# CityU-AIM-Group/HTD

Hardware: AMD Instinct MI355X
Metric: images/sec (1333x800) HTD-R50 train step (higher is better)
Workload: dtype f32; 1 GPU; HTD ResNet-50 FPN fp32 train step fwd+bwd+SGD, batch 4/GPU @ 1333x800 (padded 1344x800), random-init weights, 2000 RPN proposals/img, 512 RoIs/img/stage; global_batch=4, parallelism=dp1, stage2_positives=168, proposals=random-init RPN (few positives: the regression branch is nearly idle)

## Files before the change

htd_amd/csrc/common.h:

```cpp
#pragma once
#include <hip/hip_runtime.h>
#include <stdint.h>
#include <stdio.h>
#include <string.h>

#include "../../include/htd_amd.h"

namespace htd {

void set_error(const char *fmt, ...);
int conv_math();

inline int check_launch(const char *what)
{
    hipError_t e = hipGetLastError();
    if (e != hipSuccess) {
        set_error("%s: launch failed: %s", what, hipGetErrorString(e));
        return HTD_ERR_LAUNCH;
    }
    return HTD_OK;
}

#define HTD_REQUIRE(cond, ...)               \
    do {                                     \
        if (!(cond)) {                       \
            htd::set_error(__VA_ARGS__);     \
            return HTD_ERR_ARG;              \
        }                                    \
    } while (0)

constexpr int kWave = 64;

__device__ __forceinline__ float wave_sum(float v)
{
#pragma unroll
    for (int o = 32; o > 0; o >>= 1) v += __shfl_xor(v, o, 64);
    return v;
}
__device__ __forceinline__ float wave_max(float v)
{
#pragma unroll
    for (int o = 32; o > 0; o >>= 1) v = fmaxf(v, __shfl_xor(v, o, 64));
    return v;
}

__device__ __forceinline__ unsigned mag_bits(float v) { return (v != v) ? 0x7fc00000u : (__float_as_uint(v) & 0x7fffffffu); }
__device__ __forceinline__ unsigned mag_bits4(unsigned mx, float4 v)
{
    return max(max(mx, max(mag_bits(v.x), mag_bits(v.y))), max(mag_bits(v.z), mag_bits(v.w)));
}
__device__ __forceinline__ void wave_mag_out(unsigned bits, float *out)
{
#pragma unroll
    for (int o = 32; o > 0; o >>= 1) bits = max(bits, (unsigned)__shfl_xor((int)bits, o, 64));
    if ((threadIdx.x & 63) == 0 && bits > *reinterpret_cast<volatile unsigned *>(out))
        __hip_atomic_fetch_max(reinterpret_cast<unsigned *>(out), bits, __ATOMIC_RELAXED, __HIP_MEMORY_SCOPE_AGENT);
}

inline int64_t ceil_div(int64_t a, int64_t b) { return (a + b - 1) / b; }

}
```

htd_amd/csrc/conv_fwd.hip:

```cpp
#include <algorithm>
#include <mutex>
#include <unordered_map>

#include <stdlib.h>

#include "common.h"

namespace {

using f32x16 = __attribute__((ext_vector_type(16))) float;
using bf16x8 = __attribute__((ext_vector_type(8))) __bf16;

using bf16x2 = __attribute__((ext_vector_type(2))) __bf16;
using f32x2 = __attribute__((ext_vector_type(2))) float;

__device__ __forceinline__ void split3x2(float a, float b, unsigned &h, unsigned &m, unsigned &l)
{
    union { bf16x2 v; unsigned u; } c;
    c.v = __builtin_convertvector(f32x2{a, b}, bf16x2);
    h = c.u;
    const float ra = a - __uint_as_float(h << 16), rb = b - __uint_as_float(h & 0xffff0000u);
    c.v = __builtin_convertvector(f32x2{ra, rb}, bf16x2);
    m = c.u;
    c.v = __builtin_convertvector(f32x2{ra - __uint_as_float(m << 16), rb - __uint_as_float(m & 0xffff0000u)}, bf16x2);
// ... 383 lines not shown
                    }
                }
#pragma unroll
                for (int u = 0; u < UB; ++u)
                    if (ok[u]) {
                        *reinterpret_cast<float4 *>(p.y + o[u]) = v[u];
                        omx = htd::mag_bits4(omx, v[u]);
                    }
            }
            if (i + 1 < TM) __syncthreads();
            continue;
        }
#pragma unroll
        for (int pass = 0; pass < NPASS; ++pass) {
            const int row = tid / V + pass * RPP;
            const int64_t m = m0 + ((row >> 5) * TM + i) * 32 + (row & 31);
            if (m >= p.M || n >= p.Co) continue;
            float4 v = *reinterpret_cast<const float4 *>(lds + row * T::EPI_STRIDE + c4 * 4);
            int64_t o;
            if constexpr (TAPS) {
                const unsigned mm = (unsigned)m, wo = mm % (unsigned)p.Wo, t = mm / (unsigned)p.Wo;
                const unsigned ho = t % (unsigned)p.Ho, b = t / (unsigned)p.Ho;
                o = (((int64_t)b * p.oH + p.o_h0 + p.o_step * (int)ho) * p.oW + p.o_w0 + p.o_step * (int)wo) * p.Co + n;
            } else
                o = m * p.Co + n;
            if (tail_split >= 0) {
                const int lrow = ((row >> 5) * TM + i) * 32 + (row & 31);
                float *dst = p.partial + ((int64_t)(bid - p.tail_first) * p.tail_splits + tail_split) * (T::BM * T::BN) +
                             lrow * T::BN + c4 * 4;
                *reinterpret_cast<float4 *>(dst) = v;
                continue;
            }
            if (p.splits > 1) {
                float *dst = p.partial + (int64_t)blockIdx.y * p.M * p.Co + o;
                if (vec_ok) *reinterpret_cast<float4 *>(dst) = v;
                else {
                    dst[0] = v.x;
                    if (n + 1 < p.Co) dst[1] = v.y;
                    if (n + 2 < p.Co) dst[2] = v.z;
                    if (n + 3 < p.Co) dst[3] = v.w;
                }
                continue;
            }
            if (vec_ok) {
                if (p.bias) {
                    const float4 bv = *reinterpret_cast<const float4 *>(p.bias + n);
                    v.x += bv.x; v.y += bv.y; v.z += bv.z; v.w += bv.w;
                }
                if (p.residual) {
                    int64_t ro = o;
                    if (p.res_H > 0) {
                        const unsigned mm = (unsigned)m, wo = mm % (unsigned)p.Wo, t = mm / (unsigned)p.Wo;
                        const unsigned ho = t % (unsigned)p.Ho, b = t / (unsigned)p.Ho;
                        const int rh = min((int)floorf(ho * p.res_sh), p.res_H - 1);
                        const int rw = min((int)floorf(wo * p.res_sw), p.res_W - 1);
                        ro = (((int64_t)b * p.res_H + rh) * p.res_W + rw) * p.Co + n;
                    }
                    const float4 rv = *reinterpret_cast<const float4 *>(p.residual + ro);
                    v.x += rv.x; v.y += rv.y; v.z += rv.z; v.w += rv.w;
                }
                if (p.relu) { v.x = fmaxf(v.x, 0.f); v.y = fmaxf(v.y, 0.f); v.z = fmaxf(v.z, 0.f); v.w = fmaxf(v.w, 0.f); }
                if (p.mask_src) {
                    const float4 mv = *reinterpret_cast<const float4 *>(p.mask_src + o);
                    v.x = mv.x > 0.f ? v.x : 0.f; v.y = mv.y > 0.f ? v.y : 0.f;
                    v.z = mv.z > 0.f ? v.z : 0.f; v.w = mv.w > 0.f ? v.w : 0.f;
                }
                *reinterpret_cast<float4 *>(p.y + o) = v;
                omx = htd::mag_bits4(omx, v);
            } else {
                auto put = [&](int e, float t) {
                    if (n + e >= p.Co) return;
                    t += p.bias ? p.bias[n + e] : 0.f;
                    if (p.residual) t += p.residual[o + e];
                    if (p.relu) t = fmaxf(t, 0.f);
                    if (p.mask_src) t = p.mask_src[o + e] > 0.f ? t : 0.f;
                    p.y[o + e] = t;
                    omx = max(omx, htd::mag_bits(t));
                };
                put(0, v.x); put(1, v.y); put(2, v.z); put(3, v.w);
            }
        }
        if (i + 1 < TM) __syncthreads();
    }
    if (p.amax_out != nullptr && tail_split < 0 && p.splits <= 1) htd::wave_mag_out(omx, p.amax_out);
}

__global__ __launch_bounds__(256) void conv_splitk_epilogue_kernel(ConvParams p)
{
    const int64_t total = p.M * p.Co;
    unsigned omx = 0u;
    for (int64_t o = (int64_t)blockIdx.x * blockDim.x + threadIdx.x; o < total; o += (int64_t)gridDim.x * blockDim.x) {
        float v = 0.f;
        for (int k = 0; k < p.splits; ++k) v += p.partial[(int64_t)k * total + o];
        const int n = (int)(o % p.Co);
        if (p.bias) v += p.bias[n];
        if (p.residual) {
            int64_t ro = o;
            if (p.res_H > 0) {
                const int64_t m = o / p.Co;
                const unsigned mm = (unsigned)m, wo = mm % (unsigned)p.Wo, t = mm / (unsigned)p.Wo;
                const unsigned ho = t % (unsigned)p.Ho, b = t / (unsigned)p.Ho;
                const int rh = min((int)floorf(ho * p.res_sh), p.res_H - 1);
                const int rw = min((int)floorf(wo * p.res_sw), p.res_W - 1);
                ro = (((int64_t)b * p.res_H + rh) * p.res_W + rw) * p.Co + n;
            }
            v += p.residual[ro];
        }
        if (p.relu) v = fmaxf(v, 0.f);
        if (p.mask_src) v = p.mask_src[o] > 0.f ? v : 0.f;
        p.y[o] = v;
        omx = max(omx, htd::mag_bits(v));
    }
    if (p.amax_out != nullptr) htd::wave_mag_out(omx, p.amax_out);
}

__global__ __launch_bounds__(256) void conv_tail_epilogue_kernel(ConvParams p, int BM, int BN)
{
    const int64_t per_tile = (int64_t)BM * BN, total = (int64_t)(p.mt * p.nt - p.tail_first) * per_tile;
    unsigned omx = 0u;
    for (int64_t e = (int64_t)blockIdx.x * blockDim.x + threadIdx.x; e < total; e += (int64_t)gridDim.x * blockDim.x) {
        const int t = (int)(e / per_tile), within = (int)(e - (int64_t)t * per_tile);
        const int tile = p.tail_first + t, tile_m = tile / p.nt, tile_n = tile % p.nt;
        const int64_t m = (int64_t)tile_m * BM + within / BN;
        const int n = tile_n * BN + within % BN;
        if (m >= p.M || n >= p.Co) continue;
        const float *src = p.partial + (int64_t)t * p.tail_splits * per_tile + within;
        float v = 0.f;
        for (int k = 0; k < p.tail_splits; ++k) v += src[(int64_t)k * per_tile];
        const int64_t o = m * p.Co + n;
        if (p.bias) v += p.bias[n];
        if (p.residual) {
            int64_t ro = o;
            if (p.res_H > 0) {
                const unsigned mm = (unsigned)m, wo = mm % (unsigned)p.Wo, tt = mm / (unsigned)p.Wo;
                const unsigned ho = tt % (unsigned)p.Ho, b = tt / (unsigned)p.Ho;
                const int rh = min((int)floorf(ho * p.res_sh), p.res_H - 1);
                const int rw = min((int)floorf(wo * p.res_sw), p.res_W - 1);
                ro = (((int64_t)b * p.res_H + rh) * p.res_W + rw) * p.Co + n;
            }
            v += p.residual[ro];
        }
        if (p.relu) v = fmaxf(v, 0.f);
        if (p.mask_src) v = p.mask_src[o] > 0.f ? v : 0.f;
        p.y[o] = v;
        omx = max(omx, htd::mag_bits(v));
    }
    if (p.amax_out != nullptr) htd::wave_mag_out(omx, p.amax_out);
}

int g_conv_math = getenv("HTD_CONV_MATH") ? atoi(getenv("HTD_CONV_MATH")) : 1;

template <int WGM, int WGN, int TM, int TN>
void launch_cfg(const ConvParams &p, unsigned blocks, hipStream_t s)
{
    const dim3 grid(blocks, p.splits);
    const bool x3 = g_conv_math == 1;
    if (p.ntaps > 0) {
        if (p.Ci % 16 == 0) {
            if (x3) hipLaunchKernelGGL((conv_igemm_kernel<16, WGM, WGN, TM, TN, true, true>), grid, dim3(256), 0, s, p);
            else hipLaunchKernelGGL((conv_igemm_kernel<16, WGM, WGN, TM, TN, true>), grid, dim3(256), 0, s, p);
        } else
            hipLaunchKernelGGL((conv_igemm_kernel<8, WGM, WGN, TM, TN, true>), grid, dim3(256), 0, s, p);
    } else if (p.Ci % 32 == 0) {
        if (x3) hipLaunchKernelGGL((conv_igemm_kernel<32, WGM, WGN, TM, TN, false, true>), grid, dim3(256), 0, s, p);
        else hipLaunchKernelGGL((conv_igemm_kernel<32, WGM, WGN, TM, TN, false>), grid, dim3(256), 0, s, p);
    } else if (p.Ci % 16 == 0) {
        if (x3) hipLaunchKernelGGL((conv_igemm_kernel<16, WGM, WGN, TM, TN, false, true>), grid, dim3(256), 0, s, p);
        else hipLaunchKernelGGL((conv_igemm_kernel<16, WGM, WGN, TM, TN, false>), grid, dim3(256), 0, s, p);
    } else
        hipLaunchKernelGGL((conv_igemm_kernel<8, WGM, WGN, TM, TN, false>), grid, dim3(256), 0, s, p);
}

int plan_splits(int64_t M, int Co, int Ci, int taps)
{
    const int bk = Ci % 32 == 0 ? 32 : (Ci % 16 == 0 ? 16 : 8);
    const int total_slices = taps * (Ci / bk);
    const int64_t tiles = htd::ceil_div(M, 128) * htd::ceil_div(Co, 64);
    if (tiles <= 0 || tiles >= 384 || total_slices < 16) return 1;
    int64_t want = htd::ceil_div(768, tiles);
    want = std::min<int64_t>(want, total_slices / 8);
    return (int)std::max<int64_t>(1, std::min<int64_t>(want, 16));
}

struct TileCfg { int bm, bn; };
constexpr TileCfg kTileCfg[] = {{64, 64}, {128, 32}, {128, 64}, {128, 128}, {128, 64}, {64, 128}};
constexpr int kNumTileCfg = 6;

static const bool g_tune = getenv("HTD_CONV_TUNE") != nullptr;
int forced_tile()
{
    if (!g_tune) return -1;
    const char *e = getenv("HTD_CONV_FORCE_TILE");
    const int v = e ? atoi(e) : -1;
    return (v >= 0 && v < kNumTileCfg) ? v : -1;
}

static float tile_score(int cfg, int64_t M, int Co, int K, int splits)
{
    const int bm = kTileCfg[cfg].bm, bn = kTileCfg[cfg].bn;
    const int64_t tiles = htd::ceil_div(M, bm) * htd::ceil_div(Co, bn);
    const bool long_k = K >= 1024;
    float base;
    if (g_conv_math == 1) {
        switch (cfg) {
        case 3: base = 1.00f; break;
        case 4: base = long_k ? 0.86f : 0.90f; break;
        case 5: base = long_k ? 0.88f : 0.94f; break;
        default: base = long_k ? 0.72f : 0.82f; break;
        }
    } else {
        switch (cfg) {
        case 3: base = long_k ? 1.00f : 0.90f; break;
        case 4: base = long_k ? 0.98f : 0.97f; break;
        case 5: base = long_k ? 0.98f : 0.98f; break;
        default: base = long_k ? 0.86f : (K >= 512 ? 0.90f : 0.95f); break;
        }
    }
    const float w = (float)(tiles * splits) / 256.f;
    float quant;
    if (w >= 7.f) quant = w / ceilf(w);
    else if (w >= 3.f) quant = 0.97f;
    else quant = w / ceilf(w);
    const float useful = (float)((double)M * Co / ((double)tiles * bm * bn));
    return base * quant * useful;
}

struct TileKey {
    int64_t M;
    int Co, Ci, taps, epi;
    bool operator==(const TileKey &o) const { return M == o.M && Co == o.Co && Ci == o.Ci && taps == o.taps && epi == o.epi; }
// ... 18 lines not shown
    return it == g_tile_table.end() ? -1 : it->second;
}

int choose_tile(int64_t M, int Co, int Ci, int taps, int epi, int splits, int &bm, int &bn)
{
    const int K = taps * Ci;
    int cfg = forced_tile();
    if (cfg < 0 && epi >= 0) cfg = table_tile(M, Co, Ci, taps, epi);
    if (cfg >= 0 && Co <= 64 && kTileCfg[cfg].bn > 64) cfg = -1;
    if (cfg < 0) {
        if (Co <= 32) cfg = 1;
        else if (Co <= 64) cfg = (htd::ceil_div(M, 128) * htd::ceil_div(Co, 64) < 4400 && M >= 2048) ? 0 : 2;
        else {
            static const int cand[4] = {3, 4, 5, 0};
            float best = -1.f;
            for (int c : cand) {
                const float sc = tile_score(c, M, Co, K, splits);
                if (sc > best * 1.005f) { best = sc; cfg = c; }
            }
        }
    }
    bm = kTileCfg[cfg].bm;
    bn = kTileCfg[cfg].bn;
    return cfg;
}

static const bool g_no_tail = getenv("HTD_CONV_NO_TAIL") != nullptr;
int plan_tail(int64_t M, int Co, int Ci, int taps, int bm, int bn, int &tail_splits, int &tail_sps)
{
    tail_splits = tail_sps = 0;
    if (g_no_tail || (Co & 3)) return 0;
    const int bk = Ci % 32 == 0 ? 32 : (Ci % 16 == 0 ? 16 : 8);
    const int total_slices = taps * (Ci / bk);
    const int64_t tiles = htd::ceil_div(M, bm) * htd::ceil_div(Co, bn);
    const int64_t rem = tiles % 256, whole = tiles - rem;
    if (tiles < 256 * 3 || tiles >= 256 * 7 || rem == 0 || rem > 128 || total_slices < 8) return 0;
    int want = (int)std::min<int64_t>(16, std::max<int64_t>(2, (256 + rem / 2) / rem));
    want = std::min(want, total_slices / 4);
    if (want < 2) return 0;
    tail_sps = (int)htd::ceil_div(total_slices, want);
    tail_splits = (int)htd::ceil_div(total_slices, tail_sps);
    return (int)whole;
}

int launch_conv(ConvParams p, hipStream_t s, void *workspace)
{
    const int bk = (p.Ci % 32 == 0 && p.ntaps == 0) ? 32 : (p.Ci % 16 == 0 ? 16 : 8);
    const int total_slices = (p.ntaps > 0 ? p.ntaps : p.kh * p.kw) * (p.Ci / bk);
    p.splits = (workspace && p.ntaps == 0) ? plan_splits(p.M, p.Co, p.Ci, p.kh * p.kw) : 1;
    p.slices_per_split = (int)htd::ceil_div(total_slices, p.splits);
    p.splits = (int)htd::ceil_div(total_slices, p.slices_per_split);
    int bm, bn;
    const int epi = (p.ntaps > 0 || p.w_bstride > 0) ? -1 : ((p.residual ? 1 : 0) | (p.mask_src ? 2 : 0));
    const int cfg = choose_tile(p.M, p.Co, p.Ci, p.ntaps > 0 ? p.ntaps : p.kh * p.kw, epi, p.splits, bm, bn);
    p.mt = (int)htd::ceil_div(p.M, bm);
    p.nt = (int)htd::ceil_div(p.Co, bn);
    const int64_t blocks = (int64_t)p.mt * p.nt;
    HTD_REQUIRE(blocks > 0 && blocks < (1ll << 31), "conv2d: bad grid");
    HTD_REQUIRE((int64_t)p.B * p.Hx * p.Wx * p.Ci < (1ll << 31) && (int64_t)p.Co * p.kh * p.kw * p.Ci < (1ll << 31) &&
                    p.M < (1ll << 31),
                "conv2d: operand larger than 2^31 elements (32-bit element offsets)");
    p.partial = (float *)workspace;
    static const int cmajor_env = getenv("HTD_CONV_CMAJOR") ? atoi(getenv("HTD_CONV_CMAJOR")) : 1;
    p.cmajor = (p.ntaps == 0 && p.kh * p.kw > 1) ? cmajor_env : 0;
    unsigned launch_blocks = (unsigned)blocks;
    p.tail_first = p.tail_splits = p.tail_sps = 0;
    if (workspace && p.ntaps == 0 && p.splits == 1 && p.w_bstride == 0) {
        const int whole = plan_tail(p.M, p.Co, p.Ci, p.kh * p.kw, bm, bn, p.tail_splits, p.tail_sps);
        if (p.tail_splits > 0) {
            p.tail_first = whole;
            launch_blocks = (unsigned)(whole + (blocks - whole) * p.tail_splits);
        }
    }
    switch (cfg) {
    case 0: launch_cfg<2, 2, 1, 1>(p, launch_blocks, s); break;
    case 1: launch_cfg<4, 1, 1, 1>(p, launch_blocks, s); break;
    case 2: launch_cfg<4, 1, 1, 2>(p, launch_blocks, s); break;
    case 3: launch_cfg<2, 2, 2, 2>(p, launch_blocks, s); break;
    case 4: launch_cfg<2, 2, 2, 1>(p, launch_blocks, s); break;
    default: launch_cfg<2, 2, 1, 2>(p, launch_blocks, s); break;
    }
    if (p.tail_splits > 0) {
        const int64_t elems = (blocks - p.tail_first) * (int64_t)bm * bn;
        hipLaunchKernelGGL(conv_tail_epilogue_kernel, dim3((unsigned)htd::ceil_div(elems, 256)), dim3(256), 0, s, p, bm, bn);
    }
    if (p.splits > 1) {
        const unsigned rb = (unsigned)std::min<int64_t>(htd::ceil_div(p.M * p.Co, 256), 4096);
        hipLaunchKernelGGL(conv_splitk_epilogue_kernel, dim3(rb), dim3(256), 0, s, p);
    }
    return htd::check_launch("conv2d");
}

}

namespace htd {
int conv_math() { return g_conv_math; }
}

static int conv2d_fwd_impl(const float *x, const float *w, const float *bias, const float *residual, int res_h, int res_w, float *y,
                           int B, int H, int W, int Ci, int Co, int kh, int kw, int stride, int pad, int dil, int relu,
                           float *amax_out, void *workspace, void *stream)
{
    HTD_REQUIRE((res_h > 0) == (res_w > 0) && res_h >= 0 && (res_h == 0 || ((Co & 3) == 0 && residual)),
                "conv2d_fwd: bad residual up-sampling arguments");
    HTD_REQUIRE(B > 0 && H > 0 && W > 0 && Ci > 0 && Co > 0 && kh > 0 && kw > 0 && stride > 0 && dil > 0 && pad >= 0,
                "conv2d_fwd: bad sizes B=%d H=%d W=%d Ci=%d Co=%d k=%dx%d s=%d p=%d d=%d", B, H, W, Ci, Co, kh, kw,
                stride, pad, dil);
    HTD_REQUIRE(Ci % 8 == 0, "conv2d_fwd: Ci=%d must be a multiple of 8 (pad the stem input to 8 channels)", Ci);
    HTD_REQUIRE(x && w && y, "conv2d_fwd: null pointer");
    ConvParams p{};
    p.x = x; p.w = w; p.bias = bias; p.residual = residual; p.mask_src = nullptr; p.y = y;
    p.B = B; p.H = H; p.W = W; p.Ci = Ci; p.Co = Co; p.kh = kh; p.kw = kw; p.stride = stride; p.pad = pad; p.dil = dil;
    p.Ho = (H + 2 * pad - (dil * (kh - 1) + 1)) / stride + 1;
    p.Wo = (W + 2 * pad - (dil * (kw - 1) + 1)) / stride + 1;
    HTD_REQUIRE(p.Ho > 0 && p.Wo > 0, "conv2d_fwd: empty output");
    p.Hx = H; p.Wx = W; p.relu = relu;
    p.amax_out = amax_out;
    p.M = (int64_t)B * p.Ho * p.Wo;
    if (res_h > 0) {
        p.res_H = res_h; p.res_W = res_w;
        p.res_sh = (float)res_h / (float)p.Ho; p.res_sw = (float)res_w / (float)p.Wo;
    }
    return launch_conv(p, (hipStream_t)stream, workspace);
}

extern "C" int htd_conv2d_fwd(const float *x, const float *w, const float *bias, const float *residual, int res_h,
                              int res_w, float *y, int B, int H, int W, int Ci, int Co, int kh, int kw, int stride,
                              int pad, int dil, int relu, void *workspace, void *stream)
{
    return conv2d_fwd_impl(x, w, bias, residual, res_h, res_w, y, B, H, W, Ci, Co, kh, kw, stride, pad, dil, relu, nullptr, workspace,
                           stream);
}

extern "C" int htd_conv2d_fwd_amax(const float *x, const float *w, const float *bias, const float *residual, int res_h, int res_w,
                                   float *y, float *amax_out, int B, int H, int W, int Ci, int Co, int kh, int kw, int stride, int pad,
                                   int dil, int relu, void *workspace, void *stream)
{
    HTD_REQUIRE(amax_out, "conv2d_fwd: null maximum");
    return conv2d_fwd_impl(x, w, bias, residual, res_h, res_w, y, B, H, W, Ci, Co, kh, kw, stride, pad, dil, relu, amax_out, workspace,
                           stream);
}

extern "C" int64_t htd_conv2d_workspace_bytes(int64_t M, int Co, int Ci, int kh, int kw)
{
    const int splits = plan_splits(M, Co, Ci, kh * kw);
    if (splits > 1) return (int64_t)splits * M * Co * 4;
    int64_t need = 0;
    for (int epi = 0; epi < 4; ++epi) {
        int bm, bn, ts, tsps;
        choose_tile(M, Co, Ci, kh * kw, epi, 1, bm, bn);
        const int whole = plan_tail(M, Co, Ci, kh * kw, bm, bn, ts, tsps);
        if (ts == 0) continue;
        const int64_t tiles = htd::ceil_div(M, bm) * htd::ceil_div(Co, bn);
        need = std::max(need, (tiles - whole) * ts * (int64_t)bm * bn * 4);
    }
    return need;
}

extern "C" int htd_conv2d_tile_table_set(int64_t M, int Co, int Ci, int taps, int epi, int cfg)
{
    HTD_REQUIRE(M > 0 && Co > 0 && Ci > 0 && taps > 0 && epi >= 0 && epi < 4 && cfg < kNumTileCfg,
                "tile_table_set: bad entry M=%lld Co=%d Ci=%d taps=%d epi=%d cfg=%d", (long long)M, Co, Ci, taps, epi, cfg);
    std::lock_guard<std::mutex> lock(g_tile_mutex);
    if (cfg < 0) g_tile_table.erase(TileKey{M, Co, Ci, taps, epi});
    else g_tile_table[TileKey{M, Co, Ci, taps, epi}] = cfg;
    return HTD_OK;
}

extern "C" int htd_conv2d_tile_table_clear()
{
// ... 191 lines not shown
```

htd_amd/csrc/conv_wgrad.hip:

```cpp
#include <algorithm>

#include "common.h"

namespace {

using f32x16 = __attribute__((ext_vector_type(16))) float;

__device__ __forceinline__ float4 keep4(bool ok, float4 v)
{
    return make_float4(ok ? v.x : 0.f, ok ? v.y : 0.f, ok ? v.z : 0.f, ok ? v.w : 0.f);
}

struct WgradParams {
    const float *x, *gy;
    float *out;
    float *bias_out;
    int B, H, W, Ci, Co, kh, kw, stride, pad, dil, Ho, Wo;
    int64_t K;
    int Ntot;
    int mt, nt, splits;
    int64_t slices_per_split;
    const float *amax_x, *amax_g;
};

// ... 1174 lines not shown
    const int fcol = lane & 31, fhalf = lane >> 5;
    const int ci = ci0 + wn * 32 + fcol;
    if (ci < p.Ci) {
#pragma unroll
        for (int t = 0; t < 3; ++t) {
            const int n = (ky * 3 + t) * p.Ci + ci;
#pragma unroll
            for (int i = 0; i < TM; ++i)
#pragma unroll
                for (int r = 0; r < 16; ++r) {
                    const int m = m0 + wm * TM * 32 + i * 32 + (r & 3) + 8 * (r >> 2) + 4 * fhalf;
                    if (m < p.Co) out[(int64_t)m * p.Ntot + n] = H2 ? acc[t][i][r] * sg_inv * sx_inv : acc[t][i][r];
                }
        }
    }
}

__global__ __launch_bounds__(256) void splitk_reduce_kernel(const float *__restrict__ ws, float *__restrict__ out,
                                                            int64_t n, int splits, const float *__restrict__ ws2 = nullptr,
                                                            float *__restrict__ out2 = nullptr, int n2 = 0, int acc = 0)
{
    const int extra = out2 ? (n2 + 255) / 256 : 0;
    if ((int)blockIdx.x >= (int)gridDim.x - extra) {
        const int i = ((int)blockIdx.x - ((int)gridDim.x - extra)) * 256 + threadIdx.x;
        if (i < n2) {
            float s = acc ? out2[i] : 0.f;
            int k = 0;
            for (; k + 3 < splits; k += 4) {
                const float a = ws2[(int64_t)k * n2 + i], b = ws2[(int64_t)(k + 1) * n2 + i];
                const float c = ws2[(int64_t)(k + 2) * n2 + i], d = ws2[(int64_t)(k + 3) * n2 + i];
                s += a; s += b; s += c; s += d;
            }
            for (; k < splits; ++k) s += ws2[(int64_t)k * n2 + i];
            out2[i] = s;
        }
        return;
    }
    const unsigned main_blocks = gridDim.x - extra;
    const int64_t n4 = (n & 3) == 0 ? (n >> 2) : 0;
    for (int64_t i = (int64_t)blockIdx.x * blockDim.x + threadIdx.x; i < n4; i += (int64_t)main_blocks * blockDim.x) {
        float4 s = acc ? *reinterpret_cast<const float4 *>(out + i * 4) : make_float4(0.f, 0.f, 0.f, 0.f);
        int k = 0;
        for (; k + 3 < splits; k += 4) {
            float4 v[4];
#pragma unroll
            for (int u = 0; u < 4; ++u) v[u] = *reinterpret_cast<const float4 *>(ws + (int64_t)(k + u) * n + i * 4);
#pragma unroll
            for (int u = 0; u < 4; ++u) { s.x += v[u].x; s.y += v[u].y; s.z += v[u].z; s.w += v[u].w; }
        }
        for (; k < splits; ++k) {
            const float4 v = *reinterpret_cast<const float4 *>(ws + (int64_t)k * n + i * 4);
            s.x += v.x; s.y += v.y; s.z += v.z; s.w += v.w;
        }
        *reinterpret_cast<float4 *>(out + i * 4) = s;
    }
    if (blockIdx.x == 0)
        for (int64_t i = n4 * 4 + threadIdx.x; i < n; i += blockDim.x) {
            float s = acc ? out[i] : 0.f;
            for (int k = 0; k < splits; ++k) s += ws[(int64_t)k * n + i];
            out[i] = s;
        }
}

__global__ __launch_bounds__(256) void reduce_rows_kernel(const float *__restrict__ ws, float *__restrict__ out, int n,
                                                          int rows)
{
    __shared__ float red[16][17];
    const int col = threadIdx.x & 15, grp = threadIdx.x >> 4;
    const int c = blockIdx.x * 16 + col;
    float s = 0.f;
    if (c < n)
        for (int k = grp; k < rows; k += 16) s += ws[(int64_t)k * n + c];
    red[grp][col] = s;
    __syncthreads();
    if (grp == 0 && c < n) {
        float t = red[0][col];
#pragma unroll
        for (int g = 1; g < 16; ++g) t += red[g][col];
        out[c] = t;
    }
}

using htd::mag_bits;
using htd::wave_mag_out;

__global__ __launch_bounds__(256) void colsum_mask_kernel(const float *__restrict__ g, const float *__restrict__ y,
                                                          float *__restrict__ gm, float *__restrict__ partial,
                                                          int64_t rows, int C, int64_t rows_per_block, float *__restrict__ amax_out)
{
    const int c = blockIdx.y * 256 + threadIdx.x;
    const int64_t r0 = (int64_t)blockIdx.x * rows_per_block, r1 = min(rows, r0 + rows_per_block);
    float s = 0.f;
    unsigned mx = 0u;
    if (c < C)
        for (int64_t r = r0; r < r1; ++r) {
            float v = g[r * C + c];
            if (y) {
                v = y[r * C + c] > 0.f ? v : 0.f;
                gm[r * C + c] = v;
            }
            mx = max(mx, mag_bits(v));
            s += v;
        }
    if (amax_out) wave_mag_out(mx, amax_out);
    if (partial && c < C) partial[(int64_t)blockIdx.x * C + c] = s;
}

__global__ __launch_bounds__(256) void colsum_mask_vec_kernel(const float *__restrict__ g, const float *__restrict__ y,
                                                              float *__restrict__ gm, float *__restrict__ partial,
                                                              int64_t rows, int C, int64_t rows_per_block,
                                                              float *__restrict__ amax_out)
{
    __shared__ float4 red[256];
    unsigned mx = 0u;
    const int C4 = C >> 2;
    const int cbase = blockIdx.y * 256;
    const int cw = min(256, C4 - cbase);
    const int R = 256 / cw;
    const int c4 = threadIdx.x % cw, rsub = threadIdx.x / cw;
    const int64_t r0 = (int64_t)blockIdx.x * rows_per_block, r1 = min(rows, r0 + rows_per_block);
    float4 s = make_float4(0.f, 0.f, 0.f, 0.f);
    if (rsub < R) {
        int64_t r = r0 + rsub;
        for (; r + 3 * (int64_t)R < r1; r += 4 * (int64_t)R) {
            float4 v[4], yv[4];
#pragma unroll
            for (int u = 0; u < 4; ++u) {
                const int64_t o = (r + u * (int64_t)R) * C + (int64_t)(cbase + c4) * 4;
                v[u] = *reinterpret_cast<const float4 *>(g + o);
                if (y) yv[u] = *reinterpret_cast<const float4 *>(y + o);
            }
#pragma unroll
            for (int u = 0; u < 4; ++u) {
                if (y) {
                    const int64_t o = (r + u * (int64_t)R) * C + (int64_t)(cbase + c4) * 4;
                    v[u].x = yv[u].x > 0.f ? v[u].x : 0.f; v[u].y = yv[u].y > 0.f ? v[u].y : 0.f;
                    v[u].z = yv[u].z > 0.f ? v[u].z : 0.f; v[u].w = yv[u].w > 0.f ? v[u].w : 0.f;
                    *reinterpret_cast<float4 *>(gm + o) = v[u];
                }
                mx = htd::mag_bits4(mx, v[u]);
                s.x += v[u].x; s.y += v[u].y; s.z += v[u].z; s.w += v[u].w;
            }
        }
        for (; r < r1; r += R) {
            const int64_t o = r * C + (int64_t)(cbase + c4) * 4;
            float4 v = *reinterpret_cast<const float4 *>(g + o);
            if (y) {
                const float4 yv = *reinterpret_cast<const float4 *>(y + o);
                v.x = yv.x > 0.f ? v.x : 0.f; v.y = yv.y > 0.f ? v.y : 0.f;
                v.z = yv.z > 0.f ? v.z : 0.f; v.w = yv.w > 0.f ? v.w : 0.f;
                *reinterpret_cast<float4 *>(gm + o) = v;
            }
            mx = htd::mag_bits4(mx, v);
            s.x += v.x; s.y += v.y; s.z += v.z; s.w += v.w;
        }
    }
    if (amax_out) wave_mag_out(mx, amax_out);
    if (!partial) return;
    red[threadIdx.x] = s;
    __syncthreads();
    if (rsub == 0) {
        for (int k = 1; k < R; ++k) {
            const float4 t = red[k * cw + c4];
            s.x += t.x; s.y += t.y; s.z += t.z; s.w += t.w;
        }
        *reinterpret_cast<float4 *>(partial + (int64_t)blockIdx.x * C + (int64_t)(cbase + c4) * 4) = s;
    }
}

struct Cfg { int splits; int mt, nt; int bm, bn; };

template <int WGM, int WGN, int TM, int TN>
void launch_wgrad(int pix, bool covec, dim3 grid, hipStream_t s, const WgradParams &p)
{
#define HTD_WGRAD_CASE(PIX, CV)                                                                                   \
    if (pix == PIX && covec == CV) {                                                                               \
        hipLaunchKernelGGL((conv_wgrad_kernel<WGM, WGN, TM, TN, PIX, CV>), grid, dim3(256), 0, s, p);             \
        return;                                                                                                    \
    }
    HTD_WGRAD_CASE(PIX_POINTWISE, true) HTD_WGRAD_CASE(PIX_WIDE, true) HTD_WGRAD_CASE(PIX_GENERAL, true)
    HTD_WGRAD_CASE(PIX_POINTWISE, false) HTD_WGRAD_CASE(PIX_WIDE, false) HTD_WGRAD_CASE(PIX_GENERAL, false)
#undef HTD_WGRAD_CASE
}

Cfg choose(int Co, int Ntot, int64_t K)
{
    Cfg c;
    c.bm = Co <= 32 ? 32 : 128;
    c.bn = 128;
    c.mt = (int)htd::ceil_div(Co, c.bm);
    c.nt = (int)htd::ceil_div(Ntot, c.bn);
    const int64_t slices = htd::ceil_div(K, BKW);
    static const int units = getenv("HTD_WGRAD_UNITS") ? atoi(getenv("HTD_WGRAD_UNITS")) : 1536;
    int64_t want = htd::ceil_div(units, (int64_t)c.mt * c.nt);
    const int64_t tiles = (int64_t)c.mt * c.nt;
    int64_t cap = std::max<int64_t>(1, slices / 20);
    if (tiles * cap < 256)
        cap = std::max(cap, std::min<int64_t>(htd::ceil_div(256, tiles), std::max<int64_t>(1, slices / 5)));
    want = std::min<int64_t>(want, cap);
    c.splits = (int)std::max<int64_t>(1, std::min<int64_t>(want, 192));
    if (c.splits >= 6) c.splits = (c.splits + 7) / 8 * 8;
    static const int forced = getenv("HTD_WGRAD_SPLITS") ? atoi(getenv("HTD_WGRAD_SPLITS")) : 0;
    if (forced > 0) c.splits = (int)std::min<int64_t>(forced, slices);
    return c;
}

static const bool g_wgrad_x3h_off = getenv("HTD_WGRAD_X3H") != nullptr && atoi(getenv("HTD_WGRAD_X3H")) == 0;
bool x3h_takes(int Ci, int Co, int kh, int kw, int stride, int pad, int dil)
{
    return !g_wgrad_x3h_off && kh == 3 && kw == 3 && stride == 1 && pad == 1 && dil == 1 && Co >= 64 && (Co & 3) == 0 &&
           Ci >= 32 && (Ci & 3) == 0;
}
int x3h_splits(int B, int H, int W, int Ci, int Co)
{
    const int64_t tiles = htd::ceil_div(Co, 128) * htd::ceil_div(Ci, 64) * 3;
    const int64_t slices = htd::ceil_div((int64_t)B * H * (W + 1), XH_KS);
    static const int target = getenv("HTD_WGRAD_X3H_UNITS") ? atoi(getenv("HTD_WGRAD_X3H_UNITS")) : 768;
    int64_t want = htd::ceil_div(target, tiles);
    int64_t cap = std::max<int64_t>(1, slices / 8);
    if (tiles * cap < 256) cap = std::max(cap, std::min<int64_t>(htd::ceil_div(256, tiles), std::max<int64_t>(1, slices / 4)));
    want = std::min<int64_t>(want, cap);
    int splits = (int)std::max<int64_t>(1, std::min<int64_t>(want, 128));
    if (splits >= 6) splits = (splits + 7) / 8 * 8;
    static const int forced = getenv("HTD_WGRAD_X3H_SPLITS") ? atoi(getenv("HTD_WGRAD_X3H_SPLITS")) : 0;
    if (forced > 0) splits = (int)std::min<int64_t>(forced, std::max<int64_t>(1, slices / 2));
    return splits;
}

}

int g_wgrad_math = -1;

extern "C" int64_t htd_conv2d_wgrad_workspace_bytes(int B, int H, int W, int Ci, int Co, int kh, int kw, int stride,
                                                    int pad, int dil)
{
    const int Ho = (H + 2 * pad - (dil * (kh - 1) + 1)) / stride + 1;
    const int Wo = (W + 2 * pad - (dil * (kw - 1) + 1)) / stride + 1;
    const Cfg c = choose(Co, kh * kw * Ci, (int64_t)B * Ho * Wo);
    int splits = c.splits;
    if (x3h_takes(Ci, Co, kh, kw, stride, pad, dil)) splits = std::max(splits, x3h_splits(B, H, W, Ci, Co));
// ... 200 lines not shown
```

htd_amd/csrc/conv_x3.hip:

```cpp
#include <algorithm>
#include <mutex>
#include <type_traits>
#include <unordered_map>

#include <stdlib.h>

#include "common.h"

namespace {

using f32x16 = __attribute__((ext_vector_type(16))) float;
using bf16x8 = __attribute__((ext_vector_type(8))) __bf16;
using bf16x2 = __attribute__((ext_vector_type(2))) __bf16;
using f32x2 = __attribute__((ext_vector_type(2))) float;
using f32x4 = __attribute__((ext_vector_type(4))) float;

using f16x8 = __attribute__((ext_vector_type(8))) _Float16;
using f16x2 = __attribute__((ext_vector_type(2))) _Float16;

constexpr int XK = 16;
constexpr int NCH = 6;

struct H2Scale { float s, inv; };
__device__ __forceinline__ H2Scale h2_scale(const float *amax)
// ... 11 lines not shown
    const f32x2 back = __builtin_convertvector(c.v, f32x2);
    c.v = __builtin_convertvector(f32x2{a - back[0], b - back[1]}, f16x2);
    l = c.u;
}

__device__ __forceinline__ void split3x2(float a, float b, unsigned &h, unsigned &m, unsigned &l)
{
    union { bf16x2 v; unsigned u; } c;
    c.v = __builtin_convertvector(f32x2{a, b}, bf16x2);
    h = c.u;
    const float ra = a - __uint_as_float(h << 16), rb = b - __uint_as_float(h & 0xffff0000u);
    c.v = __builtin_convertvector(f32x2{ra, rb}, bf16x2);
    m = c.u;
    c.v = __builtin_convertvector(f32x2{ra - __uint_as_float(m << 16), rb - __uint_as_float(m & 0xffff0000u)}, bf16x2);
    l = c.u;
}

#ifndef HTD_X3P_EARLY
#define HTD_X3P_EARLY 1
#endif
#ifndef HTD_X3H_NB
#define HTD_X3H_NB 2
#endif
#ifndef HTD_X3H_FRAG_FIRST
#define HTD_X3H_FRAG_FIRST 1
#endif
#ifndef HTD_X3H_OCC4
#define HTD_X3H_OCC4 0
#endif

template <int N>
__device__ __forceinline__ void wait_vm()
{
    asm volatile("s_waitcnt vmcnt(%0)" ::"n"(N) : "memory");
}
__device__ __forceinline__ void landed(f32x4 &a) { asm volatile("" : "+v"(a)::"memory"); }

__device__ __forceinline__ void lds_dma16(const void *src, unsigned lds_dst)
{
    unsigned keep;
    asm volatile("s_mov_b32 %0, m0\n\ts_mov_b32 m0, %2\n\ts_nop 0\n\tglobal_load_lds_dwordx4 %1, off\n\ts_mov_b32 m0, %0"
                 : "=&s"(keep)
                 : "v"(src), "s"(lds_dst)
                 : "memory");
}

using u32x2 = __attribute__((ext_vector_type(2))) unsigned;
template <int OFF>
__device__ __forceinline__ void lds_store8(unsigned addr, unsigned lo, unsigned hi)
{
    const u32x2 v = {lo, hi};
    asm volatile("ds_write_b64 %0, %1 offset:%2" ::"v"(addr), "v"(v), "n"(OFF) : "memory");
}

struct X3Params {
    const float *x;
    const uint4 *wp;
    const float *bias, *residual, *mask_src;
    float *y;
    int Hx, Wx;
    int Ho, Wo;
    int Ci, Co, Cop;
    int kh;
    int stride;
    int ntl;
    int tl_dy[9], tl_dx[9], tl_w[9];
    int o_step, o_h0, o_w0, oH, oW;
    int relu;
    int res_H, res_W;
    float res_sh, res_sw;
    int64_t M;
    int mt, nt;
    int ncs;
    int tiles_a, splits_a, sps_a, splits_b, sps_b;
    int64_t m_rem0;
    float *partial;
    const uint4 *xp;
    uint4 *yp;
    int64_t xp_rows, yp_rows;
    const float *amax, *wscale;
    float *amax_out;
};

__device__ __forceinline__ void block_absmax_out(float mx, float *out, float *red, unsigned seen)
{
    unsigned bits = (mx != mx) ? 0x7fc00000u : __float_as_uint(mx);
    for (int o = 32; o > 0; o >>= 1) bits = max(bits, (unsigned)__shfl_xor((int)bits, o));
    __syncthreads();
    if ((threadIdx.x & 63) == 0) reinterpret_cast<unsigned *>(red)[threadIdx.x >> 6] = bits;
    __syncthreads();
    if (threadIdx.x == 0) {
        const unsigned *r = reinterpret_cast<const unsigned *>(red);
        bits = max(max(r[0], r[1]), max(r[2], r[3]));
        if (bits > seen) __hip_atomic_fetch_max(reinterpret_cast<unsigned *>(out), bits, __ATOMIC_RELAXED, __HIP_MEMORY_SCOPE_AGENT);
    }
}
__device__ __forceinline__ void wave_absmax_out(float mx, float *out, unsigned seen)
{
    unsigned bits = (mx != mx) ? 0x7fc00000u : __float_as_uint(mx);
    for (int o = 32; o > 0; o >>= 1) bits = max(bits, (unsigned)__shfl_xor((int)bits, o));
    if ((threadIdx.x & 63) == 0 && bits > seen)
        __hip_atomic_fetch_max(reinterpret_cast<unsigned *>(out), bits, __ATOMIC_RELAXED, __HIP_MEMORY_SCOPE_AGENT);
}
__device__ __forceinline__ float absmax4(float mx, float4 v)
{
    const float m = fmaxf(fmaxf(fabsf(v.x), fabsf(v.y)), fmaxf(fabsf(v.z), fabsf(v.w)));
    const bool nan = (v.x != v.x) | (v.y != v.y) | (v.z != v.z) | (v.w != v.w);
    return nan ? __uint_as_float(0x7fc00000u) : ((mx != mx) ? mx : fmaxf(mx, m));
}

__device__ __forceinline__ void emit_planes4(uint4 *yp, int64_t rows, int64_t m, int n, float4 v)
{
    unsigned h0, m0, l0, h1, m1, l1;
    split3x2(v.x, v.y, h0, m0, l0);
    split3x2(v.z, v.w, h1, m1, l1);
    char *d = reinterpret_cast<char *>(yp + ((int64_t)(n >> 4) * NCH + ((n >> 3) & 1)) * rows + m) + ((n >> 2) & 1) * 8;
    *reinterpret_cast<uint2 *>(d) = make_uint2(h0, h1);
    *reinterpret_cast<uint2 *>(d + 2 * rows * 16) = make_uint2(m0, m1);
    *reinterpret_cast<uint2 *>(d + 4 * rows * 16) = make_uint2(l0, l1);
}

template <int BM, int KW>
struct Geo {
    static constexpr int RUN = BM + KW - 1;
    static constexpr int PITCH = ((RUN + 1 + 3) / 8) * 8 + 4;
    static constexpr int PASSES = (RUN + 63) / 64;
};

__device__ __forceinline__ int64_t x3_out_off(const X3Params &p, int64_t m, int n)
{
    if (p.o_step == 0) return m * p.Co + n;
    const unsigned mm = (unsigned)m, wo = mm % (unsigned)p.Wo, t = mm / (unsigned)p.Wo;
    const unsigned ho = t % (unsigned)p.Ho, b = t / (unsigned)p.Ho;
    return (((int64_t)b * p.oH + p.o_h0 + p.o_step * (int)ho) * p.oW + p.o_w0 + p.o_step * (int)wo) * p.Co + n;
}

template <int WGM, int WGN, int TM, int TN, bool MF16, typename Acc>
__device__ __forceinline__ void x3_epilogue(const X3Params &p, Acc &acc, uint4 *lds, int64_t m0, int n0, bool part, bool region_b,
                                            int split)
{
    constexpr int BN = WGN * TN * 32;
    constexpr int EPI_STRIDE = BN + 4, EPI_ROWS = WGM * 32;
    constexpr int RBLK = MF16 ? 16 : 32;
    constexpr int CB = TN * 32 / RBLK;
    const int tid = threadIdx.x, lane = tid & 63, wave = tid >> 6;
    const int wm = wave / WGN, wn = wave % WGN;
    const int frow = lane & 31, fhalf = lane >> 5;
    const int lrow = MF16 ? (lane & 15) : frow;
    const int kg = lane >> 4;
    float *le = reinterpret_cast<float *>(lds);
    const bool vec_ok = (p.Co & 3) == 0;
    constexpr int V = BN / 4, RPP = 256 / V;
    float omax = 0.f;
    const unsigned oseen = (p.amax_out != nullptr && !part) ? *reinterpret_cast<const volatile unsigned *>(p.amax_out) : 0u;
    const bool scaled = p.wscale != nullptr;
    float4 cscale = make_float4(1.f, 1.f, 1.f, 1.f);
    if (scaled) {
        const float ia = h2_scale(p.amax).inv;
        const float4 w4 = *reinterpret_cast<const float4 *>(p.wscale + n0 + (tid % V) * 4);
        cscale = make_float4(w4.x * ia, w4.y * ia, w4.z * ia, w4.w * ia);
    }
#pragma unroll
    for (int i = 0; i < TM; ++i) {
        if constexpr (MF16) {
#pragma unroll
            for (int ib = 0; ib < 2; ++ib)
#pragma unroll
                for (int j = 0; j < CB; ++j)
#pragma unroll
                    for (int r = 0; r < 4; ++r)
                        le[(wm * 32 + ib * 16 + 4 * kg + r) * EPI_STRIDE + wn * TN * 32 + j * 16 + lrow] = acc[2 * i + ib][j][r];
        } else {
#pragma unroll
            for (int j = 0; j < TN; ++j)
#pragma unroll
                for (int r = 0; r < 16; ++r) {
                    const int row = wm * 32 + (r & 3) + 8 * (r >> 2) + 4 * fhalf;
                    le[row * EPI_STRIDE + (wn * TN + j) * 32 + frow] = acc[i][j][r];
                }
        }
        __syncthreads();
        const int c4 = tid % V;
        const int n = n0 + c4 * 4;
        constexpr int NPASS = EPI_ROWS / RPP;
        if (vec_ok && !part && p.res_H == 0) {
            const bool col_ok = n < p.Co;
            float4 bv = make_float4(0.f, 0.f, 0.f, 0.f);
            if (p.bias != nullptr && col_ok) bv = *reinterpret_cast<const float4 *>(p.bias + n);
            constexpr int UB = NPASS < 4 ? NPASS : 4;
#pragma unroll
            for (int pass0 = 0; pass0 < NPASS; pass0 += UB) {
                float4 v[UB], rv[UB], mv[UB];
                int64_t o[UB];
                bool ok[UB];
#pragma unroll
                for (int u = 0; u < UB; ++u) {
                    const int row = tid / V + (pass0 + u) * RPP;
                    const int64_t m = m0 + ((row >> 5) * TM + i) * 32 + (row & 31);
                    ok[u] = m < p.M && col_ok;
                    o[u] = x3_out_off(p, ok[u] ? m : 0, n) & -(int64_t)ok[u];
                    v[u] = *reinterpret_cast<const float4 *>(le + row * EPI_STRIDE + c4 * 4);
                    if (scaled) { v[u].x *= cscale.x; v[u].y *= cscale.y; v[u].z *= cscale.z; v[u].w *= cscale.w; }
                }
                if (p.residual != nullptr) {
#pragma unroll
                    for (int u = 0; u < UB; ++u) rv[u] = *reinterpret_cast<const float4 *>(p.residual + o[u]);
                }
                if (p.mask_src != nullptr) {
#pragma unroll
                    for (int u = 0; u < UB; ++u) mv[u] = *reinterpret_cast<const float4 *>(p.mask_src + o[u]);
                }
#pragma unroll
                for (int u = 0; u < UB; ++u) { v[u].x += bv.x; v[u].y += bv.y; v[u].z += bv.z; v[u].w += bv.w; }
                if (p.residual != nullptr) {
#pragma unroll
                    for (int u = 0; u < UB; ++u) { v[u].x += rv[u].x; v[u].y += rv[u].y; v[u].z += rv[u].z; v[u].w += rv[u].w; }
                }
                if (p.relu) {
#pragma unroll
                    for (int u = 0; u < UB; ++u) {
                        v[u].x = fmaxf(v[u].x, 0.f); v[u].y = fmaxf(v[u].y, 0.f); v[u].z = fmaxf(v[u].z, 0.f); v[u].w = fmaxf(v[u].w, 0.f);
                    }
                }
                if (p.mask_src != nullptr) {
#pragma unroll
                    for (int u = 0; u < UB; ++u) {
                        v[u].x = mv[u].x > 0.f ? v[u].x : 0.f; v[u].y = mv[u].y > 0.f ? v[u].y : 0.f;
                        v[u].z = mv[u].z > 0.f ? v[u].z : 0.f; v[u].w = mv[u].w > 0.f ? v[u].w : 0.f;
                    }
                }
#pragma unroll
                for (int u = 0; u < UB; ++u)
                    if (ok[u]) {
                        *reinterpret_cast<float4 *>(p.y + o[u]) = v[u];
                        omax = absmax4(omax, v[u]);
                    }
                if (p.yp != nullptr) {
#pragma unroll
                    for (int u = 0; u < UB; ++u) {
                        const int row = tid / V + (pass0 + u) * RPP;
                        if (ok[u]) emit_planes4(p.yp, p.yp_rows, m0 + ((row >> 5) * TM + i) * 32 + (row & 31), n, v[u]);
                    }
                }
            }
            if (i + 1 < TM) __syncthreads();
            continue;
        }
#pragma unroll
        for (int pass = 0; pass < NPASS; ++pass) {
            const int row = tid / V + pass * RPP;
            const int64_t m = m0 + ((row >> 5) * TM + i) * 32 + (row & 31);
            if (m >= p.M || n >= p.Co) continue;
            float4 v = *reinterpret_cast<const float4 *>(le + row * EPI_STRIDE + c4 * 4);
            if (scaled) { v.x *= cscale.x; v.y *= cscale.y; v.z *= cscale.z; v.w *= cscale.w; }
            const int64_t o = x3_out_off(p, m, n);
            if (part) {
                float *dst = region_b ? p.partial + (p.splits_a > 1 ? (int64_t)p.splits_a * p.m_rem0 * p.Co : 0) +
                                            ((int64_t)split * (p.M - p.m_rem0) + (m - p.m_rem0)) * p.Co + n
                                      : p.partial + ((int64_t)split * p.m_rem0 + m) * p.Co + n;
                if (vec_ok) *reinterpret_cast<float4 *>(dst) = v;
                else {
                    dst[0] = v.x;
                    if (n + 1 < p.Co) dst[1] = v.y;
                    if (n + 2 < p.Co) dst[2] = v.z;
                    if (n + 3 < p.Co) dst[3] = v.w;
                }
                continue;
            }
            if (vec_ok) {
                if (p.bias) {
                    const float4 bv = *reinterpret_cast<const float4 *>(p.bias + n);
                    v.x += bv.x; v.y += bv.y; v.z += bv.z; v.w += bv.w;
                }
                if (p.residual) {
                    int64_t ro = o;
                    if (p.res_H > 0) {
                        const unsigned mm = (unsigned)m, wo = mm % (unsigned)p.Wo, t = mm / (unsigned)p.Wo;
                        const unsigned ho = t % (unsigned)p.Ho, b = t / (unsigned)p.Ho;
                        const int rh = min((int)floorf(ho * p.res_sh), p.res_H - 1);
                        const int rw = min((int)floorf(wo * p.res_sw), p.res_W - 1);
                        ro = (((int64_t)b * p.res_H + rh) * p.res_W + rw) * p.Co + n;
                    }
                    const float4 rv = *reinterpret_cast<const float4 *>(p.residual + ro);
                    v.x += rv.x; v.y += rv.y; v.z += rv.z; v.w += rv.w;
                }
                if (p.relu) { v.x = fmaxf(v.x, 0.f); v.y = fmaxf(v.y, 0.f); v.z = fmaxf(v.z, 0.f); v.w = fmaxf(v.w, 0.f); }
                if (p.mask_src) {
                    const float4 mv = *reinterpret_cast<const float4 *>(p.mask_src + o);
                    v.x = mv.x > 0.f ? v.x : 0.f; v.y = mv.y > 0.f ? v.y : 0.f;
                    v.z = mv.z > 0.f ? v.z : 0.f; v.w = mv.w > 0.f ? v.w : 0.f;
                }
                *reinterpret_cast<float4 *>(p.y + o) = v;
                omax = absmax4(omax, v);
                if (p.yp != nullptr) emit_planes4(p.yp, p.yp_rows, m, n, v);
            } else {
                auto put = [&](int e, float t) {
                    if (n + e >= p.Co) return;
                    t += p.bias ? p.bias[n + e] : 0.f;
                    if (p.residual) t += p.residual[o + e];
                    if (p.relu) t = fmaxf(t, 0.f);
                    if (p.mask_src) t = p.mask_src[o + e] > 0.f ? t : 0.f;
                    p.y[o + e] = t;
                    omax = absmax4(omax, make_float4(t, 0.f, 0.f, 0.f));
                };
                put(0, v.x); put(1, v.y); put(2, v.z); put(3, v.w);
            }
        }
        if (i + 1 < TM) __syncthreads();
    }
    if (p.amax_out != nullptr && !part) block_absmax_out(omax, p.amax_out, le, oseen);
}

template <int WGM, int WGN, int TM, int TN, int KW, int NB, bool H2 = false>
constexpr int x3p_occupancy()
{
    constexpr int BM = WGM * TM * 32, BN = WGN * TN * 32;
    constexpr int NCHL = H2 ? 4 : NCH;
    constexpr int main_bytes = (2 * NCHL * Geo<BM, KW>::PITCH + NB * NCHL * BN) * 16;
    constexpr int epi_bytes = WGM * 32 * (BN + 4) * 4;
    constexpr int by_lds = 163840 / (main_bytes > epi_bytes ? main_bytes : epi_bytes);
    constexpr int by_regs = TM * TN >= 4 ? (H2 && HTD_X3H_OCC4 ? 4 : 3) : 4;
    return by_lds < by_regs ? by_lds : by_regs;
}

template <int WGM, int WGN, int TM, int TN, int KW, bool MF16, int NB, bool H2 = false>
__global__ __launch_bounds__(256, (x3p_occupancy<WGM, WGN, TM, TN, KW, NB, H2>())) void conv_x3p_kernel(X3Params p)
{
    static_assert(!(H2 && MF16), "H2: 32x32x16 form only");
    constexpr int NCHL = H2 ? 4 : NCH;
    constexpr int BM = WGM * TM * 32, BN = WGN * TN * 32;
    using G = Geo<BM, KW>;
    constexpr int PADX = (KW - 1) / 2;
    constexpr int A_VEC = NCHL * G::PITCH;
    constexpr int B_VEC = NCHL * BN;
    constexpr int MAIN_VEC = 2 * A_VEC + NB * B_VEC;
    constexpr int EPI_STRIDE = BN + 4, EPI_ROWS = WGM * 32;
    constexpr int EPI_VEC = EPI_ROWS * EPI_STRIDE / 4;
    constexpr int LDS_VEC = MAIN_VEC > EPI_VEC ? MAIN_VEC : EPI_VEC;
    __shared__ uint4 lds[LDS_VEC];
    uint4 *const lA = lds, *const lB = lds + 2 * A_VEC;
    const unsigned lds_a0 = (unsigned)(size_t)(__attribute__((address_space(3))) void *)lA;

    int bid = blockIdx.x, split = 0, sps = 0;
    bool part = false;
    const bool region_b = bid >= p.tiles_a * p.splits_a;
    if (region_b) {
        const int r = bid - p.tiles_a * p.splits_a;
        bid = p.tiles_a + r / p.splits_b;
        split = r % p.splits_b;
        part = p.splits_b > 1;
        sps = p.sps_b;
    } else if (p.splits_a > 1) {
        split = bid % p.splits_a;
        bid = bid / p.splits_a;
        part = true;
        sps = p.sps_a;
    } else {
        const int q = p.tiles_a / 8, r = p.tiles_a % 8, xcd = bid % 8, idx = bid / 8;
        bid = (xcd < r ? xcd * (q + 1) : r * (q + 1) + (xcd - r) * q) + idx;
    }
    const int tile_m = bid / p.nt, tile_n = bid % p.nt;
    const int64_t m0 = (int64_t)tile_m * BM;
    const int n0 = tile_n * BN;

    const int tid = threadIdx.x, lane = tid & 63, wave = tid >> 6;
    const int wm = wave / WGN, wn = wave % WGN;
    const int frow = lane & 31, fhalf = lane >> 5;
    const int PADY = (p.kh - 1) / 2;

    const int vcol = tid & 3, vrow = tid >> 2;
    const int a_g0 = (int)m0 + vrow - PADX;
    unsigned a_off[KW > 1 ? 1 : G::PASSES];
    bool a_in[KW > 1 ? 1 : G::PASSES];
    unsigned a_tm[KW > 1 ? 1 : G::PASSES];
    if constexpr (KW > 1) {
        a_off[0] = (unsigned)a_g0 * (unsigned)p.Ci + vcol * 4;
        a_in[0] = true;
        a_tm[0] = 0u;
    } else {
#pragma unroll
        for (int i = 0; i < G::PASSES; ++i) {
            const int64_t m = m0 + vrow + 64 * i;
            a_in[i] = vrow + 64 * i < G::RUN && m < p.M;
            const unsigned mm = a_in[i] ? (unsigned)m : 0u;
            const unsigned wo = mm % (unsigned)p.Wo, t = mm / (unsigned)p.Wo;
            const unsigned ho = t % (unsigned)p.Ho, b = t / (unsigned)p.Ho;
            a_off[i] = ((b * (unsigned)p.Hx + ho * (unsigned)p.stride) * (unsigned)p.Wx + wo * (unsigned)p.stride) *
                           (unsigned)p.Ci + vcol * 4;
            unsigned tm = 0x1ffu;
            if (p.ntl > 0) {
                tm = 0u;
                const int hb = (int)(ho * (unsigned)p.stride), wb = (int)(wo * (unsigned)p.stride);
                for (int q = 0; q < p.ntl; ++q)
// ... 462 lines not shown

    using acc_t = typename std::conditional<MF16, f32x4, f32x16>::type;
    acc_t acc[RB][CB];
#pragma unroll
    for (int i = 0; i < RB; ++i)
#pragma unroll
        for (int j = 0; j < CB; ++j)
#pragma unroll
            for (int r = 0; r < (MF16 ? 4 : 16); ++r) acc[i][j][r] = 0.f;

    auto mma = [&](int stage) __attribute__((always_inline)) {
        const char *la = reinterpret_cast<const char *>(lA + stage * A_VEC);
        const char *lb = reinterpret_cast<const char *>(lB + stage * B_VEC);
        if constexpr (MF16) {
            bf16x8 fa01[RB], fa02[RB];
#pragma unroll
            for (int i = 0; i < RB; ++i) {
                fa01[i] = *reinterpret_cast<const bf16x8 *>(la + a_c0 + i * 16 * 16);
                fa02[i] = *reinterpret_cast<const bf16x8 *>(la + a_c1 + i * 16 * 16);
            }
#pragma unroll
            for (int j = 0; j < CB; ++j) {
                const bf16x8 fb01 = *reinterpret_cast<const bf16x8 *>(lb + b_c0 + j * 16 * 16);
                const bf16x8 fb10 = *reinterpret_cast<const bf16x8 *>(lb + b_c1 + j * 16 * 16);
                const bf16x8 fb20 = *reinterpret_cast<const bf16x8 *>(lb + b_c2 + j * 16 * 16);
#pragma unroll
                for (int i = 0; i < RB; ++i) {
                    acc[i][j] = __builtin_amdgcn_mfma_f32_16x16x32_bf16(fa02[i], fb20, acc[i][j], 0, 0, 0);
                    acc[i][j] = __builtin_amdgcn_mfma_f32_16x16x32_bf16(fa01[i], fb10, acc[i][j], 0, 0, 0);
                    acc[i][j] = __builtin_amdgcn_mfma_f32_16x16x32_bf16(fa01[i], fb01, acc[i][j], 0, 0, 0);
                }
            }
        } else {
            bf16x8 fa[RB][3], fb[CB][3];
#pragma unroll
            for (int i = 0; i < RB; ++i)
#pragma unroll
                for (int q = 0; q < 3; ++q) fa[i][q] = *reinterpret_cast<const bf16x8 *>(la + a_c0 + i * 32 * 16 + q * 2 * BM * 16);
#pragma unroll
            for (int j = 0; j < CB; ++j)
#pragma unroll
                for (int q = 0; q < 3; ++q) fb[j][q] = *reinterpret_cast<const bf16x8 *>(lb + b_c0 + j * 32 * 16 + q * 2 * BN * 16);
#pragma unroll
            for (int i = 0; i < RB; ++i)
#pragma unroll
                for (int j = 0; j < CB; ++j) {
                    acc[i][j] = __builtin_amdgcn_mfma_f32_32x32x16_bf16(fa[i][2], fb[j][0], acc[i][j], 0, 0, 0);
                    acc[i][j] = __builtin_amdgcn_mfma_f32_32x32x16_bf16(fa[i][0], fb[j][2], acc[i][j], 0, 0, 0);
                    acc[i][j] = __builtin_amdgcn_mfma_f32_32x32x16_bf16(fa[i][1], fb[j][1], acc[i][j], 0, 0, 0);
                    acc[i][j] = __builtin_amdgcn_mfma_f32_32x32x16_bf16(fa[i][1], fb[j][0], acc[i][j], 0, 0, 0);
                    acc[i][j] = __builtin_amdgcn_mfma_f32_32x32x16_bf16(fa[i][0], fb[j][1], acc[i][j], 0, 0, 0);
                    acc[i][j] = __builtin_amdgcn_mfma_f32_32x32x16_bf16(fa[i][0], fb[j][0], acc[i][j], 0, 0, 0);
                }
        }
    };

    constexpr int KEEP = (NS - 2) * (NI / 4);
#pragma unroll
    for (int d = 0; d < NS - 1; ++d)
        if (s_begin + d < s_end) issue(s_begin + d, d);
    if (s_begin + NS - 2 < s_end) wait_vm<KEEP>();
    else wait_vm<0>();
    lds_barrier();
    int stage = 0, pstage = NS - 1;
#pragma unroll 1
    for (int s = s_begin; s < s_end; ++s) {
        const bool more = s + NS - 1 < s_end;
        if (more) issue(s + NS - 1, pstage);
        mma(stage);
        if (more) wait_vm<KEEP>();
        else wait_vm<0>();
        lds_barrier();
        stage = stage + 1 == NS ? 0 : stage + 1;
        pstage = pstage + 1 == NS ? 0 : pstage + 1;
    }
    x3_epilogue<WGM, WGN, TM, TN, MF16>(p, acc, lds, m0, n0, part, region_b, split);
}

__global__ __launch_bounds__(256) void conv_x3p_splitk_epilogue_kernel(X3Params p)
{
    const int64_t lo = p.splits_a > 1 ? 0 : p.m_rem0 * p.Co, hi = p.splits_b > 1 ? p.M * p.Co : p.m_rem0 * p.Co;
    const int64_t na = p.m_rem0 * p.Co, nb = (p.M - p.m_rem0) * p.Co;
    const float *pb = p.partial + (p.splits_a > 1 ? (int64_t)p.splits_a * na : 0);
    float omax = 0.f;
    const unsigned oseen = p.amax_out != nullptr ? *reinterpret_cast<const volatile unsigned *>(p.amax_out) : 0u;
    for (int64_t o = lo + (int64_t)blockIdx.x * blockDim.x + threadIdx.x; o < hi; o += (int64_t)gridDim.x * blockDim.x) {
        float v = 0.f;
        if (o < na) {
            for (int k = 0; k < p.splits_a; ++k) v += p.partial[(int64_t)k * na + o];
        } else {
            for (int k = 0; k < p.splits_b; ++k) v += pb[(int64_t)k * nb + (o - na)];
        }
        const int n = (int)(o % p.Co);
        if (p.bias) v += p.bias[n];
        if (p.residual) {
            int64_t ro = p.o_step == 0 ? o : x3_out_off(p, o / p.Co, n);
            if (p.res_H > 0) {
                const int64_t m = o / p.Co;
                const unsigned mm = (unsigned)m, wo = mm % (unsigned)p.Wo, t = mm / (unsigned)p.Wo;
                const unsigned ho = t % (unsigned)p.Ho, b = t / (unsigned)p.Ho;
                const int rh = min((int)floorf(ho * p.res_sh), p.res_H - 1);
                const int rw = min((int)floorf(wo * p.res_sw), p.res_W - 1);
                ro = (((int64_t)b * p.res_H + rh) * p.res_W + rw) * p.Co + n;
            }
            v += p.residual[ro];
        }
        if (p.relu) v = fmaxf(v, 0.f);
        const int64_t oo = p.o_step == 0 ? o : x3_out_off(p, o / p.Co, n);
        if (p.mask_src) v = p.mask_src[oo] > 0.f ? v : 0.f;
        p.y[oo] = v;
        omax = absmax4(omax, make_float4(v, 0.f, 0.f, 0.f));
    }
    __shared__ float ored[4];
    if (p.amax_out != nullptr) block_absmax_out(omax, p.amax_out, ored, oseen);
}

__global__ __launch_bounds__(256) void conv_x3p_splitk_epilogue_vec_kernel(X3Params p)
{
    const int C4 = p.Co >> 2;
    const int64_t lo = p.splits_a > 1 ? 0 : p.m_rem0 * C4, hi = p.splits_b > 1 ? p.M * C4 : p.m_rem0 * C4;
    const int64_t na = p.m_rem0 * C4, nb = (p.M - p.m_rem0) * C4;
    const float4 *pa = reinterpret_cast<const float4 *>(p.partial);
    const float4 *pb = pa + (p.splits_a > 1 ? (int64_t)p.splits_a * na : 0);
    float omax = 0.f;
    const unsigned oseen = p.amax_out != nullptr ? *reinterpret_cast<const volatile unsigned *>(p.amax_out) : 0u;
    for (int64_t q = lo + (int64_t)blockIdx.x * blockDim.x + threadIdx.x; q < hi; q += (int64_t)gridDim.x * blockDim.x) {
        float4 v = make_float4(0.f, 0.f, 0.f, 0.f);
        const bool in_a = q < na;
        const float4 *src = in_a ? pa + q : pb + (q - na);
        const int64_t stride = in_a ? na : nb;
        const int splits = in_a ? p.splits_a : p.splits_b;
#pragma unroll 4
        for (int k = 0; k < splits; ++k) {
            const float4 t = src[(int64_t)k * stride];
            v.x += t.x; v.y += t.y; v.z += t.z; v.w += t.w;
        }
        const unsigned m = (unsigned)(q / C4), n = (unsigned)(q - (int64_t)m * C4) * 4u;
        const int64_t o = x3_out_off(p, (int64_t)m, (int)n);
        if (p.bias) {
            const float4 bv = *reinterpret_cast<const float4 *>(p.bias + n);
            v.x += bv.x; v.y += bv.y; v.z += bv.z; v.w += bv.w;
        }
        if (p.residual) {
            int64_t ro = o;
            if (p.res_H > 0) {
                const unsigned wo = m % (unsigned)p.Wo, t = m / (unsigned)p.Wo;
                const unsigned ho = t % (unsigned)p.Ho, b = t / (unsigned)p.Ho;
                const int rh = min((int)floorf(ho * p.res_sh), p.res_H - 1);
                const int rw = min((int)floorf(wo * p.res_sw), p.res_W - 1);
                ro = (((int64_t)b * p.res_H + rh) * p.res_W + rw) * p.Co + n;
            }
            const float4 rv = *reinterpret_cast<const float4 *>(p.residual + ro);
            v.x += rv.x; v.y += rv.y; v.z += rv.z; v.w += rv.w;
        }
        if (p.relu) { v.x = fmaxf(v.x, 0.f); v.y = fmaxf(v.y, 0.f); v.z = fmaxf(v.z, 0.f); v.w = fmaxf(v.w, 0.f); }
        if (p.mask_src) {
            const float4 mv = *reinterpret_cast<const float4 *>(p.mask_src + o);
            v.x = mv.x > 0.f ? v.x : 0.f; v.y = mv.y > 0.f ? v.y : 0.f;
            v.z = mv.z > 0.f ? v.z : 0.f; v.w = mv.w > 0.f ? v.w : 0.f;
        }
        *reinterpret_cast<float4 *>(p.y + o) = v;
        omax = absmax4(omax, v);
        if (p.yp != nullptr) emit_planes4(p.yp, p.yp_rows, (int64_t)m, (int)n, v);
    }
    __shared__ float ored[4];
    if (p.amax_out != nullptr) block_absmax_out(omax, p.amax_out, ored, oseen);
}

__device__ __forceinline__ void x3_planes_element(const float *__restrict__ w, uint4 *__restrict__ out, int Co, int taps,
                                                  int Ci, int Np, int transposed, int64_t e)
{
    const int N = transposed ? Ci : Co, K = transposed ? Co : Ci;
    const int ncs = K / XK;
    const int n = (int)(e % Np);
    const int64_t t2 = e / Np;
    const int cs = (int)(t2 % ncs), tap = (int)(t2 / ncs);
    float v[XK];
    if (n < N) {
        if (!transposed) {
            const float4 *src = reinterpret_cast<const float4 *>(w + ((int64_t)n * taps + tap) * Ci + cs * XK);
#pragma unroll
            for (int q = 0; q < 4; ++q) {
                const float4 f = src[q];
                v[4 * q] = f.x; v[4 * q + 1] = f.y; v[4 * q + 2] = f.z; v[4 * q + 3] = f.w;
            }
        } else {
#pragma unroll
            for (int k = 0; k < XK; ++k) v[k] = w[((int64_t)(cs * XK + k) * taps + (taps - 1 - tap)) * Ci + n];
        }
    } else {
#pragma unroll
        for (int k = 0; k < XK; ++k) v[k] = 0.f;
    }
    unsigned pl[3][8];
#pragma unroll
    for (int k = 0; k < 8; ++k) split3x2(v[2 * k], v[2 * k + 1], pl[0][k], pl[1][k], pl[2][k]);
    uint4 *dst = out + ((int64_t)(tap * ncs + cs) * NCH) * Np + n;
#pragma unroll
    for (int q = 0; q < 3; ++q)
#pragma unroll
        for (int h = 0; h < 2; ++h)
            dst[(int64_t)(q * 2 + h) * Np] = make_uint4(pl[q][4 * h], pl[q][4 * h + 1], pl[q][4 * h + 2], pl[q][4 * h + 3]);
}

__global__ __launch_bounds__(256) void x3_planes_kernel(const float *__restrict__ w, uint4 *__restrict__ out, int Co, int taps,
                                                        int Ci, int Np, int transposed)
{
    const int K = transposed ? Co : Ci;
    const int64_t total = (int64_t)taps * (K / XK) * Np;
    for (int64_t e = (int64_t)blockIdx.x * 256 + threadIdx.x; e < total; e += (int64_t)gridDim.x * 256)
        x3_planes_element(w, out, Co, taps, Ci, Np, transposed, e);
}

struct PlanesDesc {
    const float *w;
    uint4 *out;
    int Co, taps, Ci, transposed;
    int64_t block0;
};

__global__ __launch_bounds__(256) void x3_planes_many_kernel(const PlanesDesc *__restrict__ descs, int n)
{
    int lo = 0, hi = n - 1;
    const int64_t b = blockIdx.x;
    while (lo < hi) {
        const int mid = (lo + hi + 1) >> 1;
        if (descs[mid].block0 <= b) lo = mid;
        else hi = mid - 1;
    }
    const PlanesDesc d = descs[lo];
    const int N = d.transposed ? d.Ci : d.Co, K = d.transposed ? d.Co : d.Ci;
    const int Np = ((N + 127) / 128) * 128;
    const int64_t total = (int64_t)d.taps * (K / XK) * Np;
    const int64_t e = (b - d.block0) * 256 + threadIdx.x;
    if (e < total) x3_planes_element(d.w, d.out, d.Co, d.taps, d.Ci, Np, d.transposed, e);
}

inline int planes_np(int N) { return (int)htd::ceil_div(N, 128) * 128; }

constexpr int H2_ECH = 1024;
__host__ __device__ inline int h2_chunks(int taps, int K) { return (taps * K + H2_ECH - 1) / H2_ECH; }

__device__ __forceinline__ void x3h_rowmax_part(const float *__restrict__ w, float *__restrict__ part, int Co, int taps, int Ci, int Np,
                                                int transposed, int n0, int chunk, float *red )
{
    const int N = transposed ? Ci : Co, K = transposed ? Co : Ci;
    const int lane = threadIdx.x & 63, wave = threadIdx.x >> 6;
    const int e0 = chunk * H2_ECH, e1 = min(taps * K, e0 + H2_ECH);
    if (transposed) {
// ... 361 lines not shown
        if (kw == 1) hipLaunchKernelGGL((conv_x3p_kernel<2, 2, TM, TN, 1, true, NB>), grid, dim3(256), 0, s, p);
        else hipLaunchKernelGGL((conv_x3p_kernel<2, 2, TM, TN, 3, true, NB>), grid, dim3(256), 0, s, p);
    }
}

template <int TM, int TN>
void launch_tile(const X3Params &p, int kw, dim3 grid, hipStream_t s)
{
#ifdef HTD_X3P_DEEP
    const int nb = x3p_nb();
    if (nb == 3) return launch_tile_nb<TM, TN, 3>(p, kw, grid, s);
    if (nb >= 4) return launch_tile_nb<TM, TN, 4>(p, kw, grid, s);
#endif
    launch_tile_nb<TM, TN, 2>(p, kw, grid, s);
}

static const int g_x3q_mfma = getenv("HTD_X3Q_MFMA") ? atoi(getenv("HTD_X3Q_MFMA")) : 0;
static const int g_x3q_ns = getenv("HTD_X3Q_NS") ? atoi(getenv("HTD_X3Q_NS")) : 0;
int x3q_env(const char *name, int at_load)
{
    if (!g_x3p_tune) return at_load;
    const char *e = getenv(name);
    return e ? atoi(e) : 0;
}

template <int TM, int TN>
void launch_tile_q(const X3Params &p, dim3 grid, hipStream_t s)
{
    const int mf = x3q_env("HTD_X3Q_MFMA", g_x3q_mfma), ns = x3q_env("HTD_X3Q_NS", g_x3q_ns);
    if (mf != 32) {
        if (ns == 3) hipLaunchKernelGGL((conv_x3q_kernel<2, 2, TM, TN, true, 3>), grid, dim3(256), 0, s, p);
        else hipLaunchKernelGGL((conv_x3q_kernel<2, 2, TM, TN, true, 2>), grid, dim3(256), 0, s, p);
    } else {
        if (ns == 3) hipLaunchKernelGGL((conv_x3q_kernel<2, 2, TM, TN, false, 3>), grid, dim3(256), 0, s, p);
        else hipLaunchKernelGGL((conv_x3q_kernel<2, 2, TM, TN, false, 2>), grid, dim3(256), 0, s, p);
    }
}

int launch_x3p(X3Params p, int kw, hipStream_t s, void *workspace)
{
    const int total_steps = p.ncs * p.kh;
    const int epi = (p.residual ? 1 : 0) | (p.mask_src ? 2 : 0) | (p.amax ? 4 : 0);
    const int cfg = choose_cfg(p.M, p.Co, p.Ci, p.kh * kw + (p.ntl > 0 ? 100 : 0), epi);
    const XPlan pl = plan_x3p(cfg, p.M, p.Co, total_steps, kw, workspace != nullptr);
    p.tiles_a = pl.tiles_a; p.splits_a = pl.splits_a; p.sps_a = pl.sps_a; p.splits_b = pl.splits_b; p.sps_b = pl.sps_b;
    p.m_rem0 = pl.m_rem0;
    p.partial = (float *)workspace;
    p.mt = (int)htd::ceil_div(p.M, kXCfg[cfg].bm);
    p.nt = (int)htd::ceil_div(p.Co, kXCfg[cfg].bn);
    HTD_REQUIRE(pl.grid > 0 && pl.grid < (1ll << 31), "conv2d_x3p: bad grid");
    const dim3 grid((unsigned)pl.grid);
    if (p.amax != nullptr && kw == 3) {
        switch (cfg) {
        case 0: hipLaunchKernelGGL((conv_x3p_kernel<2, 2, 1, 1, 3, false, HTD_X3H_NB, true>), grid, dim3(256), 0, s, p); break;
        case 1: hipLaunchKernelGGL((conv_x3p_kernel<2, 2, 2, 2, 3, false, HTD_X3H_NB, true>), grid, dim3(256), 0, s, p); break;
        case 2: hipLaunchKernelGGL((conv_x3p_kernel<2, 2, 2, 1, 3, false, HTD_X3H_NB, true>), grid, dim3(256), 0, s, p); break;
        default: hipLaunchKernelGGL((conv_x3p_kernel<2, 2, 1, 2, 3, false, HTD_X3H_NB, true>), grid, dim3(256), 0, s, p); break;
        }
    } else if (p.amax != nullptr) {
        switch (cfg) {
        case 0: hipLaunchKernelGGL((conv_x3p_kernel<2, 2, 1, 1, 1, false, HTD_X3H_NB, true>), grid, dim3(256), 0, s, p); break;
        case 1: hipLaunchKernelGGL((conv_x3p_kernel<2, 2, 2, 2, 1, false, HTD_X3H_NB, true>), grid, dim3(256), 0, s, p); break;
        case 2: hipLaunchKernelGGL((conv_x3p_kernel<2, 2, 2, 1, 1, false, HTD_X3H_NB, true>), grid, dim3(256), 0, s, p); break;
        default: hipLaunchKernelGGL((conv_x3p_kernel<2, 2, 1, 2, 1, false, HTD_X3H_NB, true>), grid, dim3(256), 0, s, p); break;
        }
    } else if (p.xp != nullptr) {
        switch (cfg) {
        case 0: launch_tile_q<1, 1>(p, grid, s); break;
        case 1: launch_tile_q<2, 2>(p, grid, s); break;
        case 2: launch_tile_q<2, 1>(p, grid, s); break;
        default: launch_tile_q<1, 2>(p, grid, s); break;
        }
    } else {
        switch (cfg) {
        case 0: launch_tile<1, 1>(p, kw, grid, s); break;
        case 1: launch_tile<2, 2>(p, kw, grid, s); break;
        case 2: launch_tile<2, 1>(p, kw, grid, s); break;
        default: launch_tile<1, 2>(p, kw, grid, s); break;
        }
    }
    if (pl.partial_floats > 0) {
        const int64_t rows = (p.splits_a > 1 ? p.m_rem0 : 0) + (p.splits_b > 1 ? p.M - p.m_rem0 : 0);
        if ((p.Co & 3) == 0) {
            const unsigned rb = (unsigned)std::min<int64_t>(htd::ceil_div(rows * (p.Co >> 2), 256), p.amax_out ? 1024 : 4096);
            hipLaunchKernelGGL(conv_x3p_splitk_epilogue_vec_kernel, dim3(rb), dim3(256), 0, s, p);
        } else {
            const unsigned rb = (unsigned)std::min<int64_t>(htd::ceil_div(rows * p.Co, 256), p.amax_out ? 1024 : 4096);
            hipLaunchKernelGGL(conv_x3p_splitk_epilogue_kernel, dim3(rb), dim3(256), 0, s, p);
        }
    }
    return htd::check_launch("conv2d_x3p");
}

bool x3h_strided_ok(int Ci, int Co, int kh, int kw, int stride, int pad)
{
    static const bool on = !(getenv("HTD_X3H_STRIDED") && atoi(getenv("HTD_X3H_STRIDED")) == 0);
    return on && Ci % XK == 0 && Co >= 33 && kh == 3 && kw == 3 && stride == 2 && pad == 1;
}

bool x3p_shape_ok(int Ci, int Co, int kh, int kw, int stride, int pad, int dil)
{
    if (Ci % XK != 0 || Co < 33 || dil != 1 || kh != kw) return false;
    if (kh == 1) return pad == 0 && stride >= 1;
    return kh == 3 && stride == 1 && pad == 1;
}

}

extern "C" int htd_conv2d_x3p_supported(int Ci, int Co, int kh, int kw, int stride, int pad, int dil)
{
    return (!x3p_off() && htd::conv_math() == 1 && x3p_shape_ok(Ci, Co, kh, kw, stride, pad, dil)) ? 1 : 0;
}

int g_conv_h2 = getenv("HTD_CONV_H2") ? atoi(getenv("HTD_CONV_H2")) : 1;
extern "C" int htd_conv2d_set_h2(int on)
{
    const int prev = g_conv_h2;
    if (on == 0 || on == 1) g_conv_h2 = on;
    return prev;
}
extern "C" int htd_conv2d_x3h_supported(int Ci, int Co, int kh, int kw, int stride, int pad, int dil)
{
    return (g_conv_h2 == 1 && htd_conv2d_x3p_supported(Ci, Co, kh, kw, stride, pad, dil)) ? 1 : 0;
}
extern "C" int htd_conv2d_x3h_strided_supported(int Ci, int Co, int kh, int kw, int stride, int pad, int dil)
{
    return (g_conv_h2 == 1 && !x3p_off() && htd::conv_math() == 1 && dil == 1 && x3h_strided_ok(Ci, Co, kh, kw, stride, pad)) ? 1 : 0;
}

extern "C" int htd_conv2d_x3p_tile_table_set(int64_t M, int Co, int Ci, int taps, int epi, int cfg)
{
    HTD_REQUIRE(M > 0 && Co > 0 && Ci > 0 && taps > 0 && epi >= 0 && epi < 8 && cfg < 4,
                "x3p_tile_table_set: bad entry M=%lld Co=%d Ci=%d taps=%d epi=%d cfg=%d", (long long)M, Co, Ci, taps, epi, cfg);
    std::lock_guard<std::mutex> lock(g_xtable_mutex);
    if (cfg < 0) g_xtable.erase(XKey{M, Co, Ci, taps, epi});
    else g_xtable[XKey{M, Co, Ci, taps, epi}] = cfg;
    return HTD_OK;
}

extern "C" int htd_conv2d_x3p_tile_table_clear()
{
    std::lock_guard<std::mutex> lock(g_xtable_mutex);
    g_xtable.clear();
    return HTD_OK;
}

extern "C" int htd_conv2d_x3p_tile_query(int64_t M, int Co, int Ci, int taps, int epi)
{
    return choose_cfg(M, Co, Ci, taps, epi);
}

extern "C" int htd_conv2d_x3p_plan_query(int cfg, int64_t M, int Co, int Ci, int kh, int kw, int64_t *out)
{
    HTD_REQUIRE(cfg >= 0 && cfg < 4 && M > 0 && Co > 0 && Ci >= XK && Ci % XK == 0 && kh > 0 && kw > 0 && out,
                "x3p_plan_query: bad arguments");
    const XPlan pl = plan_x3p(cfg, M, Co, (Ci / XK) * kh, kw, true);
    out[0] = pl.tiles_a; out[1] = pl.splits_a; out[2] = pl.sps_a; out[3] = pl.splits_b; out[4] = pl.sps_b;
    out[5] = pl.m_rem0; out[6] = pl.grid; out[7] = pl.partial_floats;
    return HTD_OK;
}

extern "C" int64_t htd_conv2d_x3_planes_bytes(int Co, int kh, int kw, int Ci, int transposed)
{
    const int N = transposed ? Ci : Co, K = transposed ? Co : Ci;
    if (N <= 0 || K <= 0 || K % XK != 0 || kh <= 0 || kw <= 0) return 0;
    return (int64_t)kh * kw * (K / XK) * NCH * planes_np(N) * 16 + (int64_t)(2 + h2_chunks(kh * kw, K)) * planes_np(N) * 4;
}

extern "C" int htd_conv2d_x3_planes(const float *w, void *planes, int Co, int kh, int kw, int Ci, int transposed, void *stream)
{
// ... 305 lines not shown
```

htd_amd/csrc/roi_align.hip:

```cpp
#include <algorithm>

#include "common.h"

namespace {

struct RoiGeom {
    float start_h, start_w, bin_h, bin_w;
    int grid_h, grid_w, batch;
    float inv_count;
};

__device__ __forceinline__ RoiGeom roi_geometry(const float *roi, float scale, int ph, int pw,
                                                int sampling_ratio, int aligned)
{
    RoiGeom g;
    const float off = aligned ? 0.5f : 0.f;
    g.batch = (int)roi[0];
    g.start_w = roi[1] * scale - off;
    g.start_h = roi[2] * scale - off;
    const float end_w = roi[3] * scale - off, end_h = roi[4] * scale - off;
    float rw = end_w - g.start_w, rh = end_h - g.start_h;
    if (!aligned) { rw = fmaxf(rw, 1.f); rh = fmaxf(rh, 1.f); }
    g.bin_h = rh / (float)ph;
    g.bin_w = rw / (float)pw;
// ... 114 lines not shown
                        if (w == 0.f) continue;
#pragma unroll
                        for (int k = 0; k < 4; ++k)
                            if (chunk * 256 + lane + 64 * k < C)
                                atomicAdd(row + (size_t)c * C + 64 * k, w * go[k]);
                    }
                }
            }
        }
    }
}

template <int WAVES>
__global__ __launch_bounds__(64 * WAVES) void roi_align_fwd_split_kernel(const float *__restrict__ feat, const float *__restrict__ rois,
                                                                  const int64_t *__restrict__ roi_level, int level,
                                                                  float *__restrict__ out, int B, int C, int H, int W, int ph,
                                                                  int pw, float scale, int sampling_ratio, int aligned,
                                                                  int chunks)
{
    __shared__ float4 part[WAVES][64];
    const int lane = threadIdx.x & 63, wave = threadIdx.x >> 6;
    const int64_t task = blockIdx.x;
    const int chunk = (int)(task % chunks);
    const int64_t t2 = task / chunks;
    const int bin = (int)(t2 % (ph * pw));
    const int64_t ri = t2 / (ph * pw);
    if (roi_level && roi_level[ri] != (int64_t)level) return;
    const int bi = bin / pw, bj = bin % pw;
    const RoiGeom g = roi_geometry(rois + 5 * ri, scale, ph, pw, sampling_ratio, aligned);
    int r0, r1, c0, c1;
    axis_span(g.start_h, g.bin_h, bi, g.grid_h, H, r0, r1);
    axis_span(g.start_w, g.bin_w, bj, g.grid_w, W, c0, c1);
    if (g.batch < 0 || g.batch >= B) { r0 = 0; r1 = -1; }
    const size_t img_base = (size_t)g.batch * H * W * C;
    const int ch = chunk * 256 + lane * 4;
    const bool act = ch < C;
    float4 acc = make_float4(0.f, 0.f, 0.f, 0.f);
    for (int rb = r0; rb <= r1; rb += 64) {
        const float wy_l = (rb + lane <= r1) ? axis_weight(g.start_h, g.bin_h, bi, g.grid_h, rb + lane, H) : 0.f;
        const int rn = min(64, r1 - rb + 1);
        for (int cb = c0; cb <= c1; cb += 64) {
            const float wx_l = (cb + lane <= c1) ? axis_weight(g.start_w, g.bin_w, bj, g.grid_w, cb + lane, W) : 0.f;
            const int cn = min(64, c1 - cb + 1);
            for (int r = wave; r < rn; r += WAVES) {
                const float wy = lane_bcast(wy_l, r);
                const float *row = feat + img_base + ((size_t)(rb + r) * W + cb) * C + ch;
#pragma unroll 4
                for (int c = 0; c < cn; ++c) {
                    const float w = wy * lane_bcast(wx_l, c);
                    if (act) {
                        const float4 v = *reinterpret_cast<const float4 *>(row + (size_t)c * C);
                        acc.x += w * v.x; acc.y += w * v.y; acc.z += w * v.z; acc.w += w * v.w;
                    }
                }
            }
        }
    }
    part[wave][lane] = acc;
    __syncthreads();
    if (wave == 0 && act) {
        float4 t = part[0][lane];
#pragma unroll
        for (int w = 1; w < WAVES; ++w) {
            const float4 v = part[w][lane];
            t.x += v.x; t.y += v.y; t.z += v.z; t.w += v.w;
        }
        t.x *= g.inv_count; t.y *= g.inv_count; t.z *= g.inv_count; t.w *= g.inv_count;
        *reinterpret_cast<float4 *>(out + ((size_t)ri * ph * pw + bin) * C + ch) = t;
    }
}

struct LevelTable {
    const float *feat[8];
    int H[8], W[8];
    float scale[8];
};

__global__ __launch_bounds__(256) void roi_align_levels_fwd_kernel(LevelTable tab, const float *__restrict__ rois,
                                                                   const int64_t *__restrict__ roi_level, float *__restrict__ out,
                                                                   int64_t n, int B, int C, int L, int ph, int pw,
                                                                   int sampling_ratio, int aligned, int chunks, int64_t tasks,
                                                                   float *__restrict__ amax_out)
{
    const int lane = threadIdx.x & 63;
    const int64_t task = (int64_t)blockIdx.x * (blockDim.x >> 6) + (threadIdx.x >> 6);
    if (task >= tasks) return;
    const unsigned seen = amax_out ? *reinterpret_cast<const volatile unsigned *>(amax_out) : 0u;
    const int chunk = (int)(task % chunks);
    const int64_t t2 = task / chunks;
    const int bin = (int)(t2 % (ph * pw));
    const int64_t ri = t2 / (ph * pw);
    const int lv = (int)roi_level[ri];
    const int ch = chunk * 256 + lane * 4;
    const bool act = ch < C;
    const size_t bin_off = ((size_t)ri * ph * pw + bin) * C;
    float4 acc = make_float4(0.f, 0.f, 0.f, 0.f);
    RoiGeom g{};
    g.inv_count = 0.f;
    if (lv >= 0 && lv < L) {
        const int H = tab.H[lv], W = tab.W[lv];
        const float *feat = tab.feat[lv];
        const int bi = bin / pw, bj = bin % pw;
        g = roi_geometry(rois + 5 * ri, tab.scale[lv], ph, pw, sampling_ratio, aligned);
        int r0, r1, c0, c1;
        axis_span(g.start_h, g.bin_h, bi, g.grid_h, H, r0, r1);
        axis_span(g.start_w, g.bin_w, bj, g.grid_w, W, c0, c1);
        if (g.batch < 0 || g.batch >= B) { r0 = 0; r1 = -1; }
        const size_t img_base = (size_t)g.batch * H * W * C;
        for (int rb = r0; rb <= r1; rb += 64) {
            const float wy_l = (rb + lane <= r1) ? axis_weight(g.start_h, g.bin_h, bi, g.grid_h, rb + lane, H) : 0.f;
            for (int cb = c0; cb <= c1; cb += 64) {
                const float wx_l = (cb + lane <= c1) ? axis_weight(g.start_w, g.bin_w, bj, g.grid_w, cb + lane, W) : 0.f;
                const int rn = min(64, r1 - rb + 1), cn = min(64, c1 - cb + 1);
                for (int r = 0; r < rn; ++r) {
                    const float wy = lane_bcast(wy_l, r);
                    const float *row = feat + img_base + ((size_t)(rb + r) * W + cb) * C + ch;
#pragma unroll 4
                    for (int c = 0; c < cn; ++c) {
                        const float w = wy * lane_bcast(wx_l, c);
                        if (act) {
                            const float4 v = *reinterpret_cast<const float4 *>(row + (size_t)c * C);
                            acc.x += w * v.x; acc.y += w * v.y; acc.z += w * v.z; acc.w += w * v.w;
                        }
                    }
                }
            }
        }
    }
    if (act) {
        acc.x *= g.inv_count; acc.y *= g.inv_count; acc.z *= g.inv_count; acc.w *= g.inv_count;
        *reinterpret_cast<float4 *>(out + bin_off + ch) = acc;
    }
    if (amax_out) {
        const bool nan = act && ((acc.x != acc.x) | (acc.y != acc.y) | (acc.z != acc.z) | (acc.w != acc.w));
        const float m = act ? fmaxf(fmaxf(fabsf(acc.x), fabsf(acc.y)), fmaxf(fabsf(acc.z), fabsf(acc.w))) : 0.f;
        unsigned bits = nan ? 0x7fc00000u : __float_as_uint(m);
        for (int o = 32; o > 0; o >>= 1) bits = max(bits, (unsigned)__shfl_xor((int)bits, o));
        if (lane == 0 && bits > seen)
            __hip_atomic_fetch_max(reinterpret_cast<unsigned *>(amax_out), bits, __ATOMIC_RELAXED, __HIP_MEMORY_SCOPE_AGENT);
    }
}

struct AllLevelsOut {
    float *out[8];
};

template <int WAVES>
__global__ __launch_bounds__(WAVES == 1 ? 256 : 64 * WAVES) void roi_align_all_levels_fwd_kernel(
    LevelTable tab, AllLevelsOut outs, const float *__restrict__ rois, int64_t n, int B, int C, int L, int ph, int pw,
    int sampling_ratio, int aligned, int chunks, int64_t tasks)
{
    __shared__ float4 part[WAVES == 1 ? 1 : WAVES][64];
    const int lane = threadIdx.x & 63, wave = threadIdx.x >> 6;
    const int64_t task = WAVES == 1 ? (int64_t)blockIdx.x * 4 + wave : (int64_t)blockIdx.x;
    if (WAVES == 1 && task >= tasks) return;
    const int chunk = (int)(task % chunks);
    int64_t t2 = task / chunks;
    const int bin = (int)(t2 % (ph * pw));
    t2 /= ph * pw;
    const int64_t ri = t2 % n;
    const int lv = (int)(t2 / n);
    const int H = tab.H[lv], W = tab.W[lv];
    const float *feat = tab.feat[lv];
    const int bi = bin / pw, bj = bin % pw;
    const RoiGeom g = roi_geometry(rois + 5 * ri, tab.scale[lv], ph, pw, sampling_ratio, aligned);
    int r0, r1, c0, c1;
    axis_span(g.start_h, g.bin_h, bi, g.grid_h, H, r0, r1);
    axis_span(g.start_w, g.bin_w, bj, g.grid_w, W, c0, c1);
    if (g.batch < 0 || g.batch >= B) { r0 = 0; r1 = -1; }
    const size_t img_base = (size_t)g.batch * H * W * C;
    const int ch = chunk * 256 + lane * 4;
    const bool act = ch < C;
    float4 acc = make_float4(0.f, 0.f, 0.f, 0.f);
    for (int rb = r0; rb <= r1; rb += 64) {
        const float wy_l = (rb + lane <= r1) ? axis_weight(g.start_h, g.bin_h, bi, g.grid_h, rb + lane, H) : 0.f;
        const int rn = min(64, r1 - rb + 1);
        for (int cb = c0; cb <= c1; cb += 64) {
            const float wx_l = (cb + lane <= c1) ? axis_weight(g.start_w, g.bin_w, bj, g.grid_w, cb + lane, W) : 0.f;
            const int cn = min(64, c1 - cb + 1);
            for (int r = (WAVES == 1 ? 0 : wave); r < rn; r += WAVES) {
                const float wy = lane_bcast(wy_l, r);
                const float *row = feat + img_base + ((size_t)(rb + r) * W + cb) * C + ch;
#pragma unroll 4
                for (int c = 0; c < cn; ++c) {
                    const float w = wy * lane_bcast(wx_l, c);
                    if (act) {
                        const float4 v = *reinterpret_cast<const float4 *>(row + (size_t)c * C);
                        acc.x += w * v.x; acc.y += w * v.y; acc.z += w * v.z; acc.w += w * v.w;
                    }
                }
            }
        }
    }
    float *dst = outs.out[lv] + ((size_t)ri * ph * pw + bin) * C + ch;
    if constexpr (WAVES == 1) {
        if (act) {
            acc.x *= g.inv_count; acc.y *= g.inv_count; acc.z *= g.inv_count; acc.w *= g.inv_count;
            *reinterpret_cast<float4 *>(dst) = acc;
        }
    } else {
        part[wave][lane] = acc;
        __syncthreads();
        if (wave == 0 && act) {
            float4 t = part[0][lane];
#pragma unroll
            for (int w = 1; w < WAVES; ++w) {
                const float4 v = part[w][lane];
                t.x += v.x; t.y += v.y; t.z += v.z; t.w += v.w;
            }
            t.x *= g.inv_count; t.y *= g.inv_count; t.z *= g.inv_count; t.w *= g.inv_count;
            *reinterpret_cast<float4 *>(dst) = t;
        }
    }
}

constexpr int MAXP = 8;

__global__ __launch_bounds__(256) void roi_align_bwd_rows_kernel(const float *__restrict__ gout,
                                                                 const float *__restrict__ rois,
                                                                 const int64_t *__restrict__ roi_level, int level,
                                                                 float *__restrict__ gfeat, int64_t n, int B, int C,
                                                                 int H, int W, int ph, int pw, float scale,
                                                                 int sampling_ratio, int aligned, int chunks,
// ... 373 lines not shown
        int r_lo, r_hi, c_lo, c_hi, t0, t1;
        axis_span(g.start_h, g.bin_h, 0, g.grid_h, H, r_lo, t0);
        axis_span(g.start_h, g.bin_h, ph - 1, g.grid_h, H, t1, r_hi);
        bool ok = g.batch >= 0 && g.batch < B && !(t0 < r_lo || r_hi < t1);
        axis_span(g.start_w, g.bin_w, 0, g.grid_w, W, c_lo, t0);
        axis_span(g.start_w, g.bin_w, pw - 1, g.grid_w, W, t1, c_hi);
        ok = ok && !(t0 < c_lo || c_hi < t1);
        if (ok) { o.b = (short)g.batch; o.r_lo = (short)r_lo; o.r_hi = (short)r_hi; o.c_lo = (short)c_lo; o.c_hi = (short)c_hi; }
    }
    const_cast<RoiBox *>(t.box[k])[ri] = o;
}

int gather_split(int64_t n, int64_t tiles_min, bool every_level)
{
    static const int forced = getenv("HTD_ROI_BWD_SPLIT") ? atoi(getenv("HTD_ROI_BWD_SPLIT")) : 0;
    if (forced == 1 || forced == 2 || forced == 4) return forced;
    (void)n; (void)tiles_min;
    return every_level ? 2 : 1;
}

int launch(bool backward, const float *in, const float *rois, const int64_t *roi_level, int level, float *out,
           int64_t n, int B, int C, int H, int W, int ph, int pw, float scale, int sr, int aligned,
           void *stream)
{
    HTD_REQUIRE(n >= 0 && B > 0 && C > 0 && H > 0 && W > 0 && ph > 0 && pw > 0,
                "roi_align: bad sizes n=%lld B=%d C=%d H=%d W=%d", (long long)n, B, C, H, W);
    HTD_REQUIRE(C % 4 == 0, "roi_align: C=%d must be a multiple of 4 (float4 channel vectors)", C);
    if (n == 0) return HTD_OK;
    HTD_REQUIRE(in && rois && out, "roi_align: null pointer");
    const int chunks = (C + 255) / 256;
    const int waves_per_block = 4;
    hipStream_t s = (hipStream_t)stream;
    if (backward && ph <= MAXP && pw <= MAXP && n * chunks >= 256) {
        const int row_slots = (int)std::min<int64_t>(H, std::max<int64_t>(8, htd::ceil_div(16384, n * chunks)));
        const int64_t tasks = n * row_slots * chunks;
        const int64_t blocks = htd::ceil_div(tasks, waves_per_block);
        HTD_REQUIRE(blocks < (1ll << 31), "roi_align: too many tasks");
        hipLaunchKernelGGL(roi_align_bwd_rows_kernel, dim3((unsigned)blocks), dim3(256), 0, s, in, rois, roi_level,
                           level, out, n, B, C, H, W, ph, pw, scale, sr, aligned, chunks, row_slots, tasks);
        return htd::check_launch("roi_align");
    }
    const int64_t tasks = n * ph * pw * chunks;
    if (!backward && tasks < 8192) {
        hipLaunchKernelGGL(roi_align_fwd_split_kernel<8>, dim3((unsigned)tasks), dim3(512), 0, s, in, rois, roi_level, level, out, B,
                           C, H, W, ph, pw, scale, sr, aligned, chunks);
        return htd::check_launch("roi_align");
    }
    const int64_t blocks = htd::ceil_div(tasks, waves_per_block);
    HTD_REQUIRE(blocks < (1ll << 31), "roi_align: too many tasks");
    if (backward)
        hipLaunchKernelGGL(roi_align_kernel<true>, dim3((unsigned)blocks), dim3(256), 0, s, in, rois, roi_level, level,
                           out, n, B, C, H, W, ph, pw, scale, sr, aligned, chunks, tasks);
    else
        hipLaunchKernelGGL(roi_align_kernel<false>, dim3((unsigned)blocks), dim3(256), 0, s, in, rois, roi_level, level,
                           out, n, B, C, H, W, ph, pw, scale, sr, aligned, chunks, tasks);
    return htd::check_launch("roi_align");
}

}

extern "C" int htd_roi_align_fwd(const float *feat, const float *rois, const int64_t *roi_level, int level,
                                 float *out, int64_t n, int B, int C, int H, int W, int ph, int pw, float spatial_scale,
                                 int sampling_ratio, int aligned, void *stream)
{
    return launch(false, feat, rois, roi_level, level, out, n, B, C, H, W, ph, pw, spatial_scale, sampling_ratio,
                  aligned, stream);
}

static int roi_align_levels_fwd_impl(const float *const *feats, const int *H, const int *W, const float *scales, int L,
                                     const float *rois, const int64_t *roi_level, float *out, int64_t n, int B, int C, int ph,
                                     int pw, int sampling_ratio, int aligned, float *amax_out, void *stream)
{
    HTD_REQUIRE(L > 0 && L <= 8 && n >= 0 && B > 0 && C > 0 && ph > 0 && pw > 0, "roi_align_levels: bad sizes");
    HTD_REQUIRE(C % 4 == 0, "roi_align_levels: C=%d must be a multiple of 4", C);
    if (n == 0) return HTD_OK;
    HTD_REQUIRE(feats && H && W && scales && rois && roi_level && out, "roi_align_levels: null pointer");
    LevelTable tab{};
    for (int l = 0; l < L; ++l) {
        HTD_REQUIRE(feats[l] && H[l] > 0 && W[l] > 0, "roi_align_levels: bad level %d", l);
        tab.feat[l] = feats[l]; tab.H[l] = H[l]; tab.W[l] = W[l]; tab.scale[l] = scales[l];
    }
    const int chunks = (C + 255) / 256;
    const int64_t tasks = n * ph * pw * chunks;
    const int64_t blocks = htd::ceil_div(tasks, 4);
    HTD_REQUIRE(blocks < (1ll << 31), "roi_align_levels: too many tasks");
    hipLaunchKernelGGL(roi_align_levels_fwd_kernel, dim3((unsigned)blocks), dim3(256), 0, (hipStream_t)stream, tab, rois, roi_level, out,
                       n, B, C, L, ph, pw, sampling_ratio, aligned, chunks, tasks, amax_out);
    return htd::check_launch("roi_align_levels");
}

extern "C" int htd_roi_align_levels_fwd(const float *const *feats, const int *H, const int *W, const float *scales, int L,
                                        const float *rois, const int64_t *roi_level, float *out, int64_t n, int B, int C, int ph,
                                        int pw, int sampling_ratio, int aligned, void *stream)
{
    return roi_align_levels_fwd_impl(feats, H, W, scales, L, rois, roi_level, out, n, B, C, ph, pw, sampling_ratio, aligned, nullptr,
                                     stream);
}

extern "C" int htd_roi_align_levels_fwd_amax(const float *const *feats, const int *H, const int *W, const float *scales, int L,
                                             const float *rois, const int64_t *roi_level, float *out, int64_t n, int B, int C,
                                             int ph, int pw, int sampling_ratio, int aligned, float *amax_out, void *stream)
{
    HTD_REQUIRE(amax_out, "roi_align_levels: null maximum");
    return roi_align_levels_fwd_impl(feats, H, W, scales, L, rois, roi_level, out, n, B, C, ph, pw, sampling_ratio, aligned, amax_out,
                                     stream);
}

extern "C" int htd_roi_align_all_levels_fwd(const float *const *feats, const int *H, const int *W, const float *scales, int L,
                                            const float *rois, float *const *outs, int64_t n, int B, int C, int ph, int pw,
                                            int sampling_ratio, int aligned, void *stream)
{
    HTD_REQUIRE(L > 0 && L <= 8 && n >= 0 && B > 0 && C > 0 && ph > 0 && pw > 0, "roi_align_all_levels: bad sizes");
    HTD_REQUIRE(C % 4 == 0, "roi_align_all_levels: C=%d must be a multiple of 4", C);
    if (n == 0) return HTD_OK;
    HTD_REQUIRE(feats && H && W && scales && rois && outs, "roi_align_all_levels: null pointer");
    LevelTable tab{};
    AllLevelsOut o{};
    for (int l = 0; l < L; ++l) {
        HTD_REQUIRE(feats[l] && outs[l] && H[l] > 0 && W[l] > 0, "roi_align_all_levels: bad level %d", l);
        tab.feat[l] = feats[l]; tab.H[l] = H[l]; tab.W[l] = W[l]; tab.scale[l] = scales[l];
        o.out[l] = outs[l];
    }
    const int chunks = (C + 255) / 256;
    const int64_t tasks = (int64_t)L * n * ph * pw * chunks;
    HTD_REQUIRE(tasks < (1ll << 31), "roi_align_all_levels: too many tasks");
    hipStream_t s = (hipStream_t)stream;
    if (tasks < 4 * 8192)
        hipLaunchKernelGGL(roi_align_all_levels_fwd_kernel<8>, dim3((unsigned)tasks), dim3(512), 0, s, tab, o, rois, n, B, C, L, ph, pw,
                           sampling_ratio, aligned, chunks, tasks);
    else
        hipLaunchKernelGGL(roi_align_all_levels_fwd_kernel<1>, dim3((unsigned)htd::ceil_div(tasks, 4)), dim3(256), 0, s, tab, o, rois, n,
                           B, C, L, ph, pw, sampling_ratio, aligned, chunks, tasks);
    return htd::check_launch("roi_align_all_levels");
}

extern "C" int64_t htd_roi_align_bwd_gather_workspace_bytes(int64_t n) { return (n > 0 ? n : 1) * (int64_t)sizeof(RoiBox); }

extern "C" int htd_roi_align_bwd_gather(const float *grad_out, const float *rois, const int64_t *roi_level, int level,
                                        float *grad_feat, int64_t n, int B, int C, int H, int W, int ph, int pw,
                                        float spatial_scale, int sampling_ratio, int aligned, int accumulate, void *workspace,
                                        void *stream)
{
    HTD_REQUIRE(n >= 0 && B > 0 && C > 0 && H > 0 && W > 0 && ph > 0 && pw > 0 && ph <= MAXP && pw <= MAXP,
                "roi_align_bwd_gather: bad sizes n=%lld B=%d C=%d H=%d W=%d out=%dx%d", (long long)n, B, C, H, W, ph, pw);
    HTD_REQUIRE(C % 4 == 0 && H < 32768 && W < 32768 && B < 32768, "roi_align_bwd_gather: C=%d must be a multiple of 4", C);
    HTD_REQUIRE(grad_feat && (n == 0 || (grad_out && rois && workspace)), "roi_align_bwd_gather: null pointer");
    hipStream_t s = (hipStream_t)stream;
    if (n == 0) {
        if (!accumulate && hipMemsetAsync(grad_feat, 0, (size_t)B * H * W * C * 4, s) != hipSuccess) {
            htd::set_error("roi_align_bwd_gather: memset failed");
            return HTD_ERR_LAUNCH;
        }
        return HTD_OK;
    }
    RoiBox *box = (RoiBox *)workspace;
    hipLaunchKernelGGL(roi_bbox_kernel, dim3((unsigned)htd::ceil_div(n, 256)), dim3(256), 0, s, rois, roi_level, level, box, n, B,
                       H, W, ph, pw, spatial_scale, sampling_ratio, aligned);
    const int segs = (W + GW_TILE - 1) / GW_TILE;
    constexpr int rows = 1;
    const int chunks = (C + 255) / 256;
    const int hts = (H + rows - 1) / rows;
    const int64_t tasks = (int64_t)B * hts * segs * chunks;
    const int64_t blocks = htd::ceil_div(tasks, 4);
    HTD_REQUIRE(blocks < (1ll << 31), "roi_align_bwd_gather: too many tiles");
    const int rs = gather_split(n, tasks, roi_level == nullptr);
    if (rs == 4)
        hipLaunchKernelGGL((roi_align_bwd_gather_kernel<4, rows, 4>), dim3((unsigned)tasks), dim3(256), 0, s, grad_out, rois, box,
                           grad_feat, n, B, C, H, W, ph, pw, spatial_scale, sampling_ratio, aligned, accumulate, chunks, segs, hts, tasks);
// ... 145 lines not shown
```

htd_amd/csrc/roi_ops.hip:

```cpp
#include <algorithm>

#include "common.h"

namespace {

__device__ __forceinline__ float4 ld4(const float *p) { return *reinterpret_cast<const float4 *>(p); }
__device__ __forceinline__ void st4(float *p, float4 v) { *reinterpret_cast<float4 *>(p) = v; }

__global__ __launch_bounds__(256) void fuse_global_fwd_kernel(const float *__restrict__ x,
                                                              const float *__restrict__ rois,
                                                              const float *__restrict__ g,
                                                              const float *__restrict__ extra, float alpha,
                                                              float *__restrict__ out, int64_t total4, int P,
                                                              int C4, int B, float *__restrict__ amax_out)
{
    unsigned mx = 0u;
    for (int64_t idx = (int64_t)blockIdx.x * blockDim.x + threadIdx.x; idx < total4;
         idx += (int64_t)gridDim.x * blockDim.x) {
        const int c4 = (int)(idx % C4);
        const int64_t i = idx / ((int64_t)P * C4);
        int b = (int)rois[5 * i];
        b = b < 0 ? 0 : (b >= B ? B - 1 : b);
        float4 v = ld4(x + idx * 4);
        const float4 gv = ld4(g + ((int64_t)b * C4 + c4) * 4);
        v.x += gv.x; v.y += gv.y; v.z += gv.z; v.w += gv.w;
        if (extra) {
            const float4 e = ld4(extra + idx * 4);
            v.x += alpha * e.x; v.y += alpha * e.y; v.z += alpha * e.z; v.w += alpha * e.w;
        }
        st4(out + idx * 4, v);
        mx = htd::mag_bits4(mx, v);
    }
    if (amax_out) htd::wave_mag_out(mx, amax_out);
}

__global__ __launch_bounds__(256) void plain_and_fused_kernel(const float *__restrict__ x, const float *__restrict__ rois,
                                                              const float *__restrict__ g, float *__restrict__ both,
                                                              int64_t total4, int P, int C4, int B, float *__restrict__ amax_out)
{
    unsigned mx = 0u;
    for (int64_t idx = (int64_t)blockIdx.x * blockDim.x + threadIdx.x; idx < total4; idx += (int64_t)gridDim.x * blockDim.x) {
        const int c4 = (int)(idx % C4);
        const int64_t i = idx / ((int64_t)P * C4);
        int b = (int)rois[5 * i];
        b = b < 0 ? 0 : (b >= B ? B - 1 : b);
        float4 v = ld4(x + idx * 4);
        st4(both + idx * 4, v);
        mx = htd::mag_bits4(mx, v);
        const float4 gv = ld4(g + ((int64_t)b * C4 + c4) * 4);
        v.x += gv.x; v.y += gv.y; v.z += gv.z; v.w += gv.w;
        st4(both + (total4 + idx) * 4, v);
        mx = htd::mag_bits4(mx, v);
    }
    if (amax_out) htd::wave_mag_out(mx, amax_out);
}

constexpr int ROIS_PER_BLOCK = 16;
__global__ __launch_bounds__(256) void fuse_global_bwd_kernel(const float *__restrict__ grad,
                                                              const float *__restrict__ rois,
                                                              float *__restrict__ gg, int64_t n, int P, int C,
                                                              int B)
{
    const int c = blockIdx.y * 256 + threadIdx.x;
    if (c >= C) return;
    const int64_t i0 = (int64_t)blockIdx.x * ROIS_PER_BLOCK;
    const int64_t i1 = min(n, i0 + ROIS_PER_BLOCK);
    float acc = 0.f;
    int cur = -1;
    for (int64_t i = i0; i < i1; ++i) {
        int b = (int)rois[5 * i];
        b = b < 0 ? 0 : (b >= B ? B - 1 : b);
        if (b != cur) {
            if (cur >= 0) atomicAdd(gg + (int64_t)cur * C + c, acc);
            acc = 0.f;
            cur = b;
        }
        const float *p = grad + (i * P) * C + c;
        for (int q = 0; q < P; ++q) acc += p[(int64_t)q * C];
    }
    if (cur >= 0) atomicAdd(gg + (int64_t)cur * C + c, acc);
}

constexpr int VROIS = 4;
__global__ __launch_bounds__(256) void fuse_global_bwd_vec_kernel(const float *__restrict__ grad,
                                                                  const float *__restrict__ rois,
                                                                  float *__restrict__ gg, int64_t n, int P, int C4,
                                                                  int B)
{
    __shared__ float4 red[4][64];
    const int lane = threadIdx.x & 63, wave = threadIdx.x >> 6;
    const int64_t i0 = (int64_t)blockIdx.x * VROIS, i1 = min(n, i0 + VROIS);
    for (int c4 = blockIdx.y * 64 + lane; c4 - lane < C4; c4 += gridDim.y * 64) {
        const bool live = c4 < C4;
        float4 acc = make_float4(0.f, 0.f, 0.f, 0.f);
        int cur = -1;
        for (int64_t i = i0; i <= i1; ++i) {
            int b = -1;
            if (i < i1) {
                b = (int)rois[5 * i];
                b = b < 0 ? 0 : (b >= B ? B - 1 : b);
            }
            if (b != cur) {
                if (cur >= 0) {
                    red[wave][lane] = acc;
                    __syncthreads();
                    if (wave == 0 && live) {
                        float4 t = red[0][lane];
                        for (int w = 1; w < 4; ++w) { t.x += red[w][lane].x; t.y += red[w][lane].y; t.z += red[w][lane].z; t.w += red[w][lane].w; }
                        float *dst = gg + ((int64_t)cur * C4 + c4) * 4;
                        atomicAdd(dst, t.x); atomicAdd(dst + 1, t.y); atomicAdd(dst + 2, t.z); atomicAdd(dst + 3, t.w);
                    }
                    __syncthreads();
                }
                acc = make_float4(0.f, 0.f, 0.f, 0.f);
                cur = b;
            }
            if (i < i1 && live) {
                const float4 *p = reinterpret_cast<const float4 *>(grad) + (i * P) * C4 + c4;
                for (int q = wave; q < P; q += 4) {
                    const float4 v = p[(int64_t)q * C4];
                    acc.x += v.x; acc.y += v.y; acc.z += v.z; acc.w += v.w;
                }
            }
        }
    }
}

struct Ptr4 { const float *p[4]; };
struct MPtr4 { float *p[4]; };

__device__ __forceinline__ void softmax4(const float *att, int L, int64_t n, int64_t i, float *w)
{
    float m = -INFINITY;
    for (int l = 0; l < L; ++l) m = fmaxf(m, att[l * n + i]);
    float s = 0.f;
    for (int l = 0; l < L; ++l) { w[l] = __expf(att[l * n + i] - m); s += w[l]; }
    const float inv = 1.f / s;
// ... 560 lines not shown
            if (d.gamma) {
                v = d.w[i] * (d.gamma[co] * rsqrtf(d.var[co] + eps));
                d.wf[i] = v;
            } else
                v = d.w[i];
        }
        tile[r][tx] = v;
    }
    if (d.gamma && t == 0 && ci_t == 0 && ty == 0 && co0 + tx < d.Co) {
        const int co = co0 + tx;
        const float s = d.gamma[co] * rsqrtf(d.var[co] + eps);
        d.bf[co] = d.beta[co] - d.mean[co] * s;
    }
    if (!d.wT) return;
    __syncthreads();
    for (int r = ty; r < 32; r += 8) {
        const int ci = ci0 + r, co = co0 + tx;
        if (ci < d.Ci && co < d.Co) d.wT[((int64_t)ci * d.taps + (d.taps - 1 - t)) * d.Co + co] = tile[tx][r];
    }
}

__global__ __launch_bounds__(256) void bn_fold_many_bwd_kernel(const FoldBwdDesc *__restrict__ descs, int n, float eps)
{
    const int l = find_layer(descs, n, (int)blockIdx.x, [](const FoldBwdDesc &x) { return x.row0; });
    const FoldBwdDesc d = descs[l];
    const int co = (int)blockIdx.x - d.row0, K = d.K;
    const float rs = rsqrtf(d.var[co] + eps);
    const float s = d.gamma[co] * rs;
    const float *wr = d.w + (int64_t)co * K, *gr = d.gwf + (int64_t)co * K;
    float *go = d.gw + (int64_t)co * K;
    float dot = 0.f;
    for (int k = threadIdx.x * 4; k < K; k += 1024) {
        const float4 v = ld4(wr + k), g = ld4(gr + k);
        dot += v.x * g.x + v.y * g.y + v.z * g.z + v.w * g.w;
        st4(go + k, make_float4(g.x * s, g.y * s, g.z * s, g.w * s));
    }
    __shared__ float red[4];
    dot = htd::wave_sum(dot);
    if ((threadIdx.x & 63) == 0) red[threadIdx.x >> 6] = dot;
    __syncthreads();
    if (threadIdx.x == 0) {
        const float tot = red[0] + red[1] + red[2] + red[3];
        const float gb = d.gbf[co];
        d.gbeta[co] = gb;
        d.ggamma[co] = (tot - d.mean[co] * gb) * rs;
    }
}

__global__ __launch_bounds__(256) void rows_gather_kernel(const float4 *__restrict__ x, const int64_t *__restrict__ rows,
                                                          float4 *__restrict__ out, int64_t total, int F4)
{
    for (int64_t t = (int64_t)blockIdx.x * 256 + threadIdx.x; t < total; t += (int64_t)gridDim.x * 256) {
        const int64_t i = t / F4;
        out[t] = x[rows[i] * F4 + (t - i * F4)];
    }
}
__global__ __launch_bounds__(256) void rows_add_kernel(const float4 *__restrict__ g, const int64_t *__restrict__ rows,
                                                       float4 *__restrict__ gx, int64_t total, int F4)
{
    for (int64_t t = (int64_t)blockIdx.x * 256 + threadIdx.x; t < total; t += (int64_t)gridDim.x * 256) {
        const int64_t i = t / F4;
        const int64_t o = rows[i] * F4 + (t - i * F4);
        const float4 a = gx[o], b = g[t];
        gx[o] = make_float4(a.x + b.x, a.y + b.y, a.z + b.z, a.w + b.w);
    }
}

inline unsigned grid_for(int64_t work, int block = 256, int cap = 4096)
{
    int64_t b = htd::ceil_div(work, block);
    return (unsigned)(b < 1 ? 1 : (b > cap ? cap : b));
}

}

static int fuse_global_fwd_impl(const float *roi_feats, const float *rois, const float *global_feat, const float *extra, float alpha,
                                float *out, int64_t n, int P, int C, int B, float *amax_out, void *stream)
{
    HTD_REQUIRE(C % 4 == 0 && P > 0 && B > 0 && n >= 0, "fuse_global: bad sizes n=%lld P=%d C=%d B=%d",
                (long long)n, P, C, B);
    if (n == 0) return HTD_OK;
    HTD_REQUIRE(roi_feats && rois && global_feat && out, "fuse_global: null pointer");
    const int64_t total4 = n * P * (C / 4);
    hipLaunchKernelGGL(fuse_global_fwd_kernel, dim3(grid_for(total4)), dim3(256), 0, (hipStream_t)stream, roi_feats,
                       rois, global_feat, extra, alpha, out, total4, P, C / 4, B, amax_out);
    return htd::check_launch("fuse_global_fwd");
}

extern "C" int htd_fuse_global_fwd(const float *roi_feats, const float *rois, const float *global_feat,
                                   const float *extra, float alpha, float *out, int64_t n, int P, int C, int B,
                                   void *stream)
{
    return fuse_global_fwd_impl(roi_feats, rois, global_feat, extra, alpha, out, n, P, C, B, nullptr, stream);
}

extern "C" int htd_fuse_global_fwd_amax(const float *roi_feats, const float *rois, const float *global_feat, const float *extra,
                                        float alpha, float *out, int64_t n, int P, int C, int B, float *amax_out, void *stream)
{
    HTD_REQUIRE(amax_out, "fuse_global: null maximum");
    return fuse_global_fwd_impl(roi_feats, rois, global_feat, extra, alpha, out, n, P, C, B, amax_out, stream);
}

static int plain_and_fused_impl(const float *roi_feats, const float *rois, const float *global_feat, float *both, int64_t n, int P,
                                int C, int B, float *amax_out, void *stream)
{
    HTD_REQUIRE(C % 4 == 0 && P > 0 && B > 0 && n >= 0, "plain_and_fused: bad sizes n=%lld P=%d C=%d B=%d", (long long)n, P, C, B);
    if (n == 0) return HTD_OK;
    HTD_REQUIRE(roi_feats && rois && global_feat && both, "plain_and_fused: null pointer");
    const int64_t total4 = n * P * (C / 4);
    hipLaunchKernelGGL(plain_and_fused_kernel, dim3(grid_for(total4)), dim3(256), 0, (hipStream_t)stream, roi_feats, rois,
                       global_feat, both, total4, P, C / 4, B, amax_out);
    return htd::check_launch("plain_and_fused_fwd");
}

extern "C" int htd_plain_and_fused_fwd(const float *roi_feats, const float *rois, const float *global_feat, float *both,
                                       int64_t n, int P, int C, int B, void *stream)
{
    return plain_and_fused_impl(roi_feats, rois, global_feat, both, n, P, C, B, nullptr, stream);
}

extern "C" int htd_plain_and_fused_fwd_amax(const float *roi_feats, const float *rois, const float *global_feat, float *both,
                                            int64_t n, int P, int C, int B, float *amax_out, void *stream)
{
    HTD_REQUIRE(amax_out, "plain_and_fused: null maximum");
    return plain_and_fused_impl(roi_feats, rois, global_feat, both, n, P, C, B, amax_out, stream);
}

extern "C" int htd_fuse_global_bwd_global(const float *grad, const float *rois, float *grad_global, int64_t n, int P,
                                          int C, int B, void *stream)
{
    HTD_REQUIRE(P > 0 && C > 0 && B > 0 && n >= 0, "fuse_global_bwd: bad sizes");
    if (n == 0) return HTD_OK;
    HTD_REQUIRE(grad && rois && grad_global, "fuse_global_bwd: null pointer");
    if ((C & 3) == 0 && (((uintptr_t)grad | (uintptr_t)grad_global) & 15) == 0) {
        dim3 grid((unsigned)htd::ceil_div(n, VROIS), (unsigned)htd::ceil_div(C / 4, 64));
        hipLaunchKernelGGL(fuse_global_bwd_vec_kernel, grid, dim3(256), 0, (hipStream_t)stream, grad, rois,
                           grad_global, n, P, C / 4, B);
        return htd::check_launch("fuse_global_bwd");
    }
    dim3 grid((unsigned)htd::ceil_div(n, ROIS_PER_BLOCK), (unsigned)htd::ceil_div(C, 256));
    hipLaunchKernelGGL(fuse_global_bwd_kernel, grid, dim3(256), 0, (hipStream_t)stream, grad, rois, grad_global, n, P,
                       C, B);
    return htd::check_launch("fuse_global_bwd");
}

extern "C" int htd_fuse_global_bwd_global_ws(const float *grad, const float *rois, float *grad_global, int64_t n, int P,
                                             int C, int B, void *workspace, void *stream)
{
    HTD_REQUIRE(P > 0 && C > 0 && B > 0 && n >= 0 && (C & 3) == 0, "fuse_global_bwd_ws: bad sizes");
    HTD_REQUIRE(grad_global, "fuse_global_bwd_ws: null pointer");
    hipStream_t s = (hipStream_t)stream;
    if (n == 0) {
        hipMemsetAsync(grad_global, 0, (size_t)B * C * 4, s);
        return HTD_OK;
    }
    HTD_REQUIRE(grad && rois && workspace, "fuse_global_bwd_ws: null pointer");
    float *tile = (float *)workspace, *partial = tile + n * C;
    const int chunks = (int)htd::ceil_div(n, IMG_CHUNK);
    hipLaunchKernelGGL(roi_tile_sums_kernel, dim3((unsigned)n), dim3(256), 0, s, grad, tile, P, C / 4);
    hipLaunchKernelGGL(image_sums_kernel, dim3((unsigned)B, (unsigned)htd::ceil_div(C / 4, 64), (unsigned)chunks), dim3(64), 0, s,
                       (const float *)tile, rois, partial, n, C / 4, B);
    hipLaunchKernelGGL(chunk_sums_kernel, dim3((unsigned)htd::ceil_div((int64_t)B * C, 256)), dim3(256), 0, s,
                       (const float *)partial, grad_global, (int64_t)B * C, chunks);
    return htd::check_launch("fuse_global_bwd_ws");
}

extern "C" int htd_ba_fuse_fwd(const float *const *lvl, int L, const float *border, const float *att, float *out,
                               int64_t n, int ph, int pw, int C, int edge, void *stream)
{
    HTD_REQUIRE(L >= 1 && L <= 4, "ba_fuse: L=%d not in [1,4]", L);
    HTD_REQUIRE(C % 4 == 0 && ph > 0 && pw > 0 && edge >= 0, "ba_fuse: bad sizes");
    if (n == 0) return HTD_OK;
    HTD_REQUIRE(lvl && border && att && out, "ba_fuse: null pointer");
    Ptr4 p{};
    for (int l = 0; l < L; ++l) p.p[l] = lvl[l];
    hipLaunchKernelGGL(ba_fuse_fwd_kernel, dim3((unsigned)n), dim3(256), 0, (hipStream_t)stream, p, L, border, att,
                       out, n, ph, pw, C / 4, edge);
    return htd::check_launch("ba_fuse_fwd");
}

extern "C" int htd_ba_fuse_bwd(const float *const *lvl, int L, const float *att, const float *grad_out,
                               float *const *grad_lvl, float *grad_border, float *grad_att, int64_t n, int ph, int pw,
                               int C, int edge, void *stream)
{
    HTD_REQUIRE(L >= 1 && L <= 4, "ba_fuse: L=%d not in [1,4]", L);
    HTD_REQUIRE(C % 4 == 0 && ph > 0 && pw > 0 && edge >= 0, "ba_fuse: bad sizes");
    if (n == 0) return HTD_OK;
    HTD_REQUIRE(lvl && att && grad_out && grad_lvl && grad_att, "ba_fuse_bwd: null pointer");
    Ptr4 p{};
    MPtr4 g{};
    for (int l = 0; l < L; ++l) { p.p[l] = lvl[l]; g.p[l] = grad_lvl[l]; }
    hipLaunchKernelGGL(ba_fuse_bwd_kernel, dim3((unsigned)n), dim3(256), 0, (hipStream_t)stream, p, L, att, grad_out,
                       g, grad_border, grad_att, n, ph, pw, C / 4, edge);
// ... 133 lines not shown
extern "C" int htd_sgd_momentum_step(float *param, const float *grad, float *momentum_buf, int64_t n,
                                     const float *lr_dev, float momentum, float weight_decay, float grad_scale,
                                     void *stream)
{
    if (n == 0) return HTD_OK;
    HTD_REQUIRE(param && grad && momentum_buf && lr_dev, "sgd: null pointer");
    HTD_REQUIRE((((uintptr_t)param | (uintptr_t)grad | (uintptr_t)momentum_buf) & 15) == 0,
                "sgd: buffers must be 16-byte aligned");
    hipLaunchKernelGGL(sgd_kernel, dim3(grid_for(n / 4 + 1)), dim3(256), 0, (hipStream_t)stream, param, grad,
                       momentum_buf, n, lr_dev, momentum, weight_decay, grad_scale);
    return htd::check_launch("sgd");
}

__global__ __launch_bounds__(64) void log_accumulate_kernel(const float *__restrict__ packed, int n, int loss_index,
                                                            float weight, int64_t iter, double *__restrict__ acc)
{
    const double w = (double)weight;
    for (int i = threadIdx.x; i < n; i += 64)
        acc[i] = __dadd_rn(acc[i], __dmul_rn(w, (double)packed[i]));
    if (threadIdx.x == 0) {
        acc[n] = __dadd_rn(acc[n], w);
        if (!isfinite(packed[loss_index]) && acc[n + 1] < 0.0) acc[n + 1] = (double)iter;
    }
}

extern "C" int htd_log_accumulate(const float *packed, int n, int loss_index, float weight, int64_t iter, double *acc,
                                  void *stream)
{
    HTD_REQUIRE(n > 0 && loss_index >= 0 && loss_index < n, "log_accumulate: n=%d loss_index=%d", n, loss_index);
    HTD_REQUIRE(iter >= 0, "log_accumulate: iter=%lld", (long long)iter);
    HTD_REQUIRE(packed && acc, "log_accumulate: null pointer");
    hipLaunchKernelGGL(log_accumulate_kernel, dim3(1), dim3(64), 0, (hipStream_t)stream, packed, n, loss_index, weight,
                       iter, acc);
    return htd::check_launch("log_accumulate");
}

extern "C" int htd_bn_fold_fwd(const float *w, const float *gamma, const float *beta, const float *mean,
                               const float *var, float eps, float *w_folded, float *b_folded, int Co, int K,
                               void *stream)
{
    HTD_REQUIRE(Co > 0 && K > 0 && K % 4 == 0, "bn_fold: bad sizes Co=%d K=%d", Co, K);
    HTD_REQUIRE(w && gamma && beta && mean && var && w_folded && b_folded, "bn_fold: null pointer");
    hipLaunchKernelGGL(bn_fold_fwd_kernel, dim3((unsigned)Co), dim3(256), 0, (hipStream_t)stream, w, gamma, beta, mean,
                       var, eps, w_folded, b_folded, K);
    return htd::check_launch("bn_fold_fwd");
}

extern "C" int htd_bn_fold_many_fwd(const void *desc, int n_layers, int total_tiles, float eps, void *stream)
{
    static_assert(sizeof(FoldDesc) == 80, "FoldDesc layout is part of the ABI");
    HTD_REQUIRE(desc && n_layers > 0 && total_tiles > 0, "bn_fold_many_fwd: bad arguments");
    hipLaunchKernelGGL(bn_fold_many_fwd_kernel, dim3((unsigned)total_tiles), dim3(256), 0, (hipStream_t)stream,
                       (const FoldDesc *)desc, n_layers, eps);
    return htd::check_launch("bn_fold_many_fwd");
}

extern "C" int htd_bn_fold_many_bwd(const void *desc, int n_layers, int total_rows, float eps, void *stream)
{
    static_assert(sizeof(FoldBwdDesc) == 88, "FoldBwdDesc layout is part of the ABI");
    HTD_REQUIRE(desc && n_layers > 0 && total_rows > 0, "bn_fold_many_bwd: bad arguments");
    hipLaunchKernelGGL(bn_fold_many_bwd_kernel, dim3((unsigned)total_rows), dim3(256), 0, (hipStream_t)stream,
                       (const FoldBwdDesc *)desc, n_layers, eps);
    return htd::check_launch("bn_fold_many_bwd");
}

extern "C" int htd_bn_fold_bwd(const float *w, const float *gamma, const float *mean, const float *var, float eps,
                               const float *gw_folded, const float *gb_folded, float *gw, float *ggamma, float *gbeta,
                               int Co, int K, void *stream)
{
    HTD_REQUIRE(Co > 0 && K > 0 && K % 4 == 0, "bn_fold: bad sizes Co=%d K=%d", Co, K);
    HTD_REQUIRE(w && gamma && mean && var && gw_folded && gb_folded && gw && ggamma && gbeta, "bn_fold_bwd: null pointer");
    hipLaunchKernelGGL(bn_fold_bwd_kernel, dim3((unsigned)Co), dim3(256), 0, (hipStream_t)stream, w, gamma, mean, var,
                       eps, gw_folded, gb_folded, gw, ggamma, gbeta, K);
    return htd::check_launch("bn_fold_bwd");
}

namespace {

__global__ __launch_bounds__(256) void max_pool_fwd_kernel(const float *__restrict__ x, float *__restrict__ y,
                                                           int *__restrict__ idx, int B, int H, int W, int C4, int Ho,
                                                           int Wo, int k, int s, int p, float *__restrict__ amax_out)
{
    const int64_t total = (int64_t)B * Ho * Wo * C4;
    unsigned mx = 0u;
    for (int64_t t = (int64_t)blockIdx.x * 256 + threadIdx.x; t < total; t += (int64_t)gridDim.x * 256) {
        const int c4 = (int)(t % C4);
        int64_t r = t / C4;
        const int wo = (int)(r % Wo);
        r /= Wo;
        const int ho = (int)(r % Ho), b = (int)(r / Ho);
        float4 m = make_float4(-INFINITY, -INFINITY, -INFINITY, -INFINITY);
        int4 am = make_int4(-1, -1, -1, -1);
        for (int i = 0; i < k; ++i) {
            const int hi = ho * s - p + i;
            if ((unsigned)hi >= (unsigned)H) continue;
            for (int j = 0; j < k; ++j) {
                const int wi = wo * s - p + j;
                if ((unsigned)wi >= (unsigned)W) continue;
                const float4 v = reinterpret_cast<const float4 *>(x)[(((int64_t)b * H + hi) * W + wi) * C4 + c4];
                const int pix = hi * W + wi;
                if (v.x > m.x || v.x != v.x) { m.x = v.x; am.x = pix; }
                if (v.y > m.y || v.y != v.y) { m.y = v.y; am.y = pix; }
                if (v.z > m.z || v.z != v.z) { m.z = v.z; am.z = pix; }
                if (v.w > m.w || v.w != v.w) { m.w = v.w; am.w = pix; }
            }
        }
        reinterpret_cast<float4 *>(y)[t] = m;
        if (idx) reinterpret_cast<int4 *>(idx)[t] = am;
        mx = htd::mag_bits4(mx, m);
    }
    if (amax_out) htd::wave_mag_out(mx, amax_out);
}

__global__ __launch_bounds__(256) void max_pool_bwd_kernel(const float *__restrict__ g, const int *__restrict__ idx,
                                                           float *__restrict__ gx, int B, int H, int W, int C4, int Ho,
                                                           int Wo, int k, int s, int p)
{
    const int64_t total = (int64_t)B * H * W * C4;
    for (int64_t t = (int64_t)blockIdx.x * 256 + threadIdx.x; t < total; t += (int64_t)gridDim.x * 256) {
        const int c4 = (int)(t % C4);
        int64_t r = t / C4;
        const int wi = (int)(r % W);
        r /= W;
        const int hi = (int)(r % H), b = (int)(r / H);
        const int pix = hi * W + wi;
        float4 acc = make_float4(0.f, 0.f, 0.f, 0.f);
        const int ho_lo = max(0, (hi + p - k + s) / s), ho_hi = min(Ho - 1, (hi + p) / s);
        const int wo_lo = max(0, (wi + p - k + s) / s), wo_hi = min(Wo - 1, (wi + p) / s);
        for (int ho = ho_lo; ho <= ho_hi; ++ho)
            for (int wo = wo_lo; wo <= wo_hi; ++wo) {
                const int64_t o = (((int64_t)b * Ho + ho) * Wo + wo) * C4 + c4;
                const int4 am = reinterpret_cast<const int4 *>(idx)[o];
                const float4 gv = reinterpret_cast<const float4 *>(g)[o];
                if (am.x == pix) acc.x += gv.x;
                if (am.y == pix) acc.y += gv.y;
                if (am.z == pix) acc.z += gv.z;
                if (am.w == pix) acc.w += gv.w;
            }
        reinterpret_cast<float4 *>(gx)[t] = acc;
    }
}

}

namespace {
__global__ __launch_bounds__(256) void upsample_nearest_bwd_kernel(const float4 *__restrict__ g, float4 *__restrict__ out, int B,
                                                                   int H, int W, int h, int w, int C4, float sh, float sw)
{
    const int64_t total = (int64_t)B * h * w * C4;
    for (int64_t e = (int64_t)blockIdx.x * 256 + threadIdx.x; e < total; e += (int64_t)gridDim.x * 256) {
        const int c = (int)(e % C4);
        int64_t t = e / C4;
        const int rw = (int)(t % w);
        t /= w;
        const int rh = (int)(t % h), b = (int)(t / h);
        const int ho0 = max(0, (int)floorf(rh / sh) - 1), ho1 = min(H - 1, (int)ceilf((rh + 1) / sh) + 1);
        const int wo0 = max(0, (int)floorf(rw / sw) - 1), wo1 = min(W - 1, (int)ceilf((rw + 1) / sw) + 1);
        float4 acc = make_float4(0.f, 0.f, 0.f, 0.f);
        for (int ho = ho0; ho <= ho1; ++ho) {
            if (min((int)floorf(ho * sh), h - 1) != rh) continue;
            for (int wo = wo0; wo <= wo1; ++wo) {
                if (min((int)floorf(wo * sw), w - 1) != rw) continue;
                const float4 v = g[(((int64_t)b * H + ho) * W + wo) * C4 + c];
                acc.x += v.x; acc.y += v.y; acc.z += v.z; acc.w += v.w;
            }
        }
        out[e] = acc;
    }
}
}

namespace {
__global__ __launch_bounds__(256) void upsample_nearest_bwd_bf16_kernel(const uint2 *__restrict__ g, uint2 *__restrict__ out, int B,
                                                                        int H, int W, int h, int w, int C4, float sh, float sw)
{
    const int64_t total = (int64_t)B * h * w * C4;
    for (int64_t e = (int64_t)blockIdx.x * 256 + threadIdx.x; e < total; e += (int64_t)gridDim.x * 256) {
        const int c = (int)(e % C4);
        int64_t t = e / C4;
        const int rw = (int)(t % w);
        t /= w;
        const int rh = (int)(t % h), b = (int)(t / h);
        const int ho0 = max(0, (int)floorf(rh / sh) - 1), ho1 = min(H - 1, (int)ceilf((rh + 1) / sh) + 1);
        const int wo0 = max(0, (int)floorf(rw / sw) - 1), wo1 = min(W - 1, (int)ceilf((rw + 1) / sw) + 1);
        float acc[4] = {0.f, 0.f, 0.f, 0.f};
        for (int ho = ho0; ho <= ho1; ++ho) {
            if (min((int)floorf(ho * sh), h - 1) != rh) continue;
            for (int wo = wo0; wo <= wo1; ++wo) {
                if (min((int)floorf(wo * sw), w - 1) != rw) continue;
                const uint2 v = g[(((int64_t)b * H + ho) * W + wo) * C4 + c];
                acc[0] += __uint_as_float(v.x << 16); acc[1] += __uint_as_float(v.x & 0xffff0000u);
                acc[2] += __uint_as_float(v.y << 16); acc[3] += __uint_as_float(v.y & 0xffff0000u);
            }
        }
        unsigned r[4];
#pragma unroll
        for (int k = 0; k < 4; ++k) {
            const unsigned u = __float_as_uint(acc[k]);
            r[k] = (u & 0x7fffffffu) > 0x7f800000u ? ((u >> 16) | 0x40u) : ((u + 0x7fffu + ((u >> 16) & 1u)) >> 16);
        }
        out[e] = make_uint2(r[0] | (r[1] << 16), r[2] | (r[3] << 16));
    }
}
}

extern "C" int htd_upsample_nearest_bwd_bf16(const void *g, void *out, int B, int H, int W, int h, int w, int C, void *stream)
{
    HTD_REQUIRE(g && out && B > 0 && H > 0 && W > 0 && h > 0 && w > 0 && C > 0 && C % 4 == 0,
                "upsample_nearest_bwd_bf16: bad arguments");
    const int64_t total = (int64_t)B * h * w * (C / 4);
    const unsigned blocks = (unsigned)std::min<int64_t>(htd::ceil_div(total, 256), 65536);
    hipLaunchKernelGGL(upsample_nearest_bwd_bf16_kernel, dim3(blocks), dim3(256), 0, (hipStream_t)stream, (const uint2 *)g,
                       (uint2 *)out, B, H, W, h, w, C / 4, (float)h / (float)H, (float)w / (float)W);
    return htd::check_launch("upsample_nearest_bwd_bf16");
}

extern "C" int htd_upsample_nearest_bwd(const float *g, float *out, int B, int H, int W, int h, int w, int C, void *stream)
{
    HTD_REQUIRE(g && out && B > 0 && H > 0 && W > 0 && h > 0 && w > 0 && C > 0 && C % 4 == 0, "upsample_nearest_bwd: bad arguments");
    const int64_t total = (int64_t)B * h * w * (C / 4);
    const unsigned blocks = (unsigned)std::min<int64_t>(htd::ceil_div(total, 256), 65536);
    hipLaunchKernelGGL(upsample_nearest_bwd_kernel, dim3(blocks), dim3(256), 0, (hipStream_t)stream, (const float4 *)g,
                       (float4 *)out, B, H, W, h, w, C / 4, (float)h / (float)H, (float)w / (float)W);
    return htd::check_launch("upsample_nearest_bwd");
}

static int max_pool2d_fwd_impl(const float *x, float *y, int *idx, int B, int H, int W, int C, int k, int stride, int pad,
                               float *amax_out, void *stream)
{
    HTD_REQUIRE(B > 0 && H > 0 && W > 0 && C > 0 && k > 0 && stride > 0 && pad >= 0 && 2 * pad <= k,
                "max_pool2d: bad sizes");
    HTD_REQUIRE(C % 4 == 0, "max_pool2d: C=%d must be a multiple of 4", C);
    HTD_REQUIRE((int64_t)H * W < (1ll << 31), "max_pool2d: map too large");
    HTD_REQUIRE(x && y, "max_pool2d: null pointer");
    const int Ho = (H + 2 * pad - k) / stride + 1, Wo = (W + 2 * pad - k) / stride + 1;
    HTD_REQUIRE(Ho > 0 && Wo > 0, "max_pool2d: empty output");
    const int64_t total = (int64_t)B * Ho * Wo * (C / 4);
    const unsigned blocks = (unsigned)std::min<int64_t>(htd::ceil_div(total, 256), 65536);
    hipLaunchKernelGGL(max_pool_fwd_kernel, dim3(blocks), dim3(256), 0, (hipStream_t)stream, x, y, idx, B, H, W, C / 4,
                       Ho, Wo, k, stride, pad, amax_out);
    return htd::check_launch("max_pool2d_fwd");
}

extern "C" int htd_max_pool2d_fwd(const float *x, float *y, int *idx, int B, int H, int W, int C, int k, int stride,
                                  int pad, void *stream)
{
    return max_pool2d_fwd_impl(x, y, idx, B, H, W, C, k, stride, pad, nullptr, stream);
}

extern "C" int htd_max_pool2d_fwd_amax(const float *x, float *y, int *idx, int B, int H, int W, int C, int k, int stride, int pad,
                                       float *amax_out, void *stream)
{
    HTD_REQUIRE(amax_out, "max_pool2d: null maximum");
    return max_pool2d_fwd_impl(x, y, idx, B, H, W, C, k, stride, pad, amax_out, stream);
}

extern "C" int htd_max_pool2d_bwd(const float *g, const int *idx, float *gx, int B, int H, int W, int C, int k,
                                  int stride, int pad, void *stream)
{
    HTD_REQUIRE(B > 0 && H > 0 && W > 0 && C > 0 && k > 0 && stride > 0 && pad >= 0 && C % 4 == 0,
                "max_pool2d_bwd: bad sizes");
    HTD_REQUIRE(g && idx && gx, "max_pool2d_bwd: null pointer");
    const int Ho = (H + 2 * pad - k) / stride + 1, Wo = (W + 2 * pad - k) / stride + 1;
    const int64_t total = (int64_t)B * H * W * (C / 4);
    const unsigned blocks = (unsigned)std::min<int64_t>(htd::ceil_div(total, 256), 65536);
    hipLaunchKernelGGL(max_pool_bwd_kernel, dim3(blocks), dim3(256), 0, (hipStream_t)stream, g, idx, gx, B, H, W, C / 4,
                       Ho, Wo, k, stride, pad);
    return htd::check_launch("max_pool2d_bwd");
}

extern "C" int htd_rows_gather(const float *x, const int64_t *rows, float *out, int64_t n, int64_t N, int F, void *stream)
{
    HTD_REQUIRE(n >= 0 && N >= 0 && F > 0 && F % 4 == 0, "rows_gather: bad sizes n=%lld N=%lld F=%d", (long long)n, (long long)N, F);
    if (n == 0) return HTD_OK;
    HTD_REQUIRE(x && rows && out, "rows_gather: null pointer");
    const int64_t total = n * (F / 4);
    hipLaunchKernelGGL(rows_gather_kernel, dim3(grid_for(total, 256, 8192)), dim3(256), 0, (hipStream_t)stream, (const float4 *)x, rows,
                       (float4 *)out, total, F / 4);
    return htd::check_launch("rows_gather");
}

extern "C" int htd_rows_add(const float *g, const int64_t *rows, float *gx, int64_t n, int64_t N, int F, void *stream)
{
    HTD_REQUIRE(n >= 0 && N >= 0 && F > 0 && F % 4 == 0, "rows_add: bad sizes n=%lld N=%lld F=%d", (long long)n, (long long)N, F);
    if (n == 0) return HTD_OK;
    HTD_REQUIRE(g && rows && gx, "rows_add: null pointer");
    const int64_t total = n * (F / 4);
    hipLaunchKernelGGL(rows_add_kernel, dim3(grid_for(total, 256, 8192)), dim3(256), 0, (hipStream_t)stream, (const float4 *)g, rows,
                       (float4 *)gx, total, F / 4);
    return htd::check_launch("rows_add");
}
```

Measured before the change: 124.0 images/sec.

## Reduce abs-max atomics to one per block and cap emit grids

Replaces the per-wave atomic max on the activation abs-max scalar with a block-level LDS reduction followed by a single atomic from thread 0, skipping it when the value is zero. Grids of the epilogue, pool, fuse and roi-align kernels are capped and made grid-stride, so fewer blocks contend on the same atomic. NaN handling in the magnitude encoding is dropped, and the roi-align kernel is rewritten as a persistent loop. The aim is to remove contention on the global atomic. The cost is an extra __syncthreads per block, and a NaN now encodes as a large magnitude rather than the canonical value.

Measured after the change: 122.5 images/sec. 1.2% lower.

```diff
diff --git a/htd_amd/csrc/common.h b/htd_amd/csrc/common.h
--- a/htd_amd/csrc/common.h
+++ b/htd_amd/csrc/common.h
@@ -44,17 +44,24 @@
     return v;
 }
 
-__device__ __forceinline__ unsigned mag_bits(float v) { return (v != v) ? 0x7fc00000u : (__float_as_uint(v) & 0x7fffffffu); }
+constexpr int kEmitGrid = 2048;
+__device__ __forceinline__ unsigned mag_bits(float v) { return __float_as_uint(v) & 0x7fffffffu; }
 __device__ __forceinline__ unsigned mag_bits4(unsigned mx, float4 v)
 {
     return max(max(mx, max(mag_bits(v.x), mag_bits(v.y))), max(mag_bits(v.z), mag_bits(v.w)));
 }
-__device__ __forceinline__ void wave_mag_out(unsigned bits, float *out)
+__device__ __forceinline__ void block_mag_out(unsigned bits, float *out, unsigned *red)
 {
 #pragma unroll
     for (int o = 32; o > 0; o >>= 1) bits = max(bits, (unsigned)__shfl_xor((int)bits, o, 64));
-    if ((threadIdx.x & 63) == 0 && bits > *reinterpret_cast<volatile unsigned *>(out))
-        __hip_atomic_fetch_max(reinterpret_cast<unsigned *>(out), bits, __ATOMIC_RELAXED, __HIP_MEMORY_SCOPE_AGENT);
+    if ((threadIdx.x & 63) == 0) red[threadIdx.x >> 6] = bits;
+    __syncthreads();
+    if (threadIdx.x == 0) {
+        const int nw = (int)(blockDim.x + 63) >> 6;
+        for (int w = 1; w < nw; ++w) bits = max(bits, red[w]);
+        if (bits != 0u)
+            __hip_atomic_fetch_max(reinterpret_cast<unsigned *>(out), bits, __ATOMIC_RELAXED, __HIP_MEMORY_SCOPE_AGENT);
+    }
 }
 
 inline int64_t ceil_div(int64_t a, int64_t b) { return (a + b - 1) / b; }
diff --git a/htd_amd/csrc/conv_fwd.hip b/htd_amd/csrc/conv_fwd.hip
--- a/htd_amd/csrc/conv_fwd.hip
+++ b/htd_amd/csrc/conv_fwd.hip
@@ -489,11 +489,15 @@
         }
         if (i + 1 < TM) __syncthreads();
     }
-    if (p.amax_out != nullptr && tail_split < 0 && p.splits <= 1) htd::wave_mag_out(omx, p.amax_out);
+    if (p.amax_out != nullptr && tail_split < 0 && p.splits <= 1) {
+        __syncthreads();
+        htd::block_mag_out(omx, p.amax_out, reinterpret_cast<unsigned *>(lds));
+    }
 }
 
 __global__ __launch_bounds__(256) void conv_splitk_epilogue_kernel(ConvParams p)
 {
+    __shared__ unsigned mxs[4];
     const int64_t total = p.M * p.Co;
     unsigned omx = 0u;
     for (int64_t o = (int64_t)blockIdx.x * blockDim.x + threadIdx.x; o < total; o += (int64_t)gridDim.x * blockDim.x) {
@@ -518,12 +522,13 @@
         p.y[o] = v;
         omx = max(omx, htd::mag_bits(v));
     }
-    if (p.amax_out != nullptr) htd::wave_mag_out(omx, p.amax_out);
+    if (p.amax_out != nullptr) htd::block_mag_out(omx, p.amax_out, mxs);
 }
 
 __global__ __launch_bounds__(256) void conv_tail_epilogue_kernel(ConvParams p, int BM, int BN)
 {
     const int64_t per_tile = (int64_t)BM * BN, total = (int64_t)(p.mt * p.nt - p.tail_first) * per_tile;
+    __shared__ unsigned mxs[4];
     unsigned omx = 0u;
     for (int64_t e = (int64_t)blockIdx.x * blockDim.x + threadIdx.x; e < total; e += (int64_t)gridDim.x * blockDim.x) {
         const int t = (int)(e / per_tile), within = (int)(e - (int64_t)t * per_tile);
@@ -552,7 +557,7 @@
         p.y[o] = v;
         omx = max(omx, htd::mag_bits(v));
     }
-    if (p.amax_out != nullptr) htd::wave_mag_out(omx, p.amax_out);
+    if (p.amax_out != nullptr) htd::block_mag_out(omx, p.amax_out, mxs);
 }
 
 int g_conv_math = getenv("HTD_CONV_MATH") ? atoi(getenv("HTD_CONV_MATH")) : 1;
@@ -737,10 +742,11 @@
     }
     if (p.tail_splits > 0) {
         const int64_t elems = (blocks - p.tail_first) * (int64_t)bm * bn;
-        hipLaunchKernelGGL(conv_tail_epilogue_kernel, dim3((unsigned)htd::ceil_div(elems, 256)), dim3(256), 0, s, p, bm, bn);
+        hipLaunchKernelGGL(conv_tail_epilogue_kernel, dim3((unsigned)std::min<int64_t>(htd::ceil_div(elems, 256), htd::kEmitGrid)), dim3(256), 0, s,
+                           p, bm, bn);
     }
     if (p.splits > 1) {
-        const unsigned rb = (unsigned)std::min<int64_t>(htd::ceil_div(p.M * p.Co, 256), 4096);
+        const unsigned rb = (unsigned)std::min<int64_t>(htd::ceil_div(p.M * p.Co, 256), htd::kEmitGrid);
         hipLaunchKernelGGL(conv_splitk_epilogue_kernel, dim3(rb), dim3(256), 0, s, p);
     }
     return htd::check_launch("conv2d");
diff --git a/htd_amd/csrc/conv_wgrad.hip b/htd_amd/csrc/conv_wgrad.hip
--- a/htd_amd/csrc/conv_wgrad.hip
+++ b/htd_amd/csrc/conv_wgrad.hip
@@ -1280,7 +1280,7 @@
 }
 
 using htd::mag_bits;
-using htd::wave_mag_out;
+using htd::block_mag_out;
 
 __global__ __launch_bounds__(256) void colsum_mask_kernel(const float *__restrict__ g, const float *__restrict__ y,
                                                           float *__restrict__ gm, float *__restrict__ partial,
@@ -1288,6 +1288,7 @@
 {
     const int c = blockIdx.y * 256 + threadIdx.x;
     const int64_t r0 = (int64_t)blockIdx.x * rows_per_block, r1 = min(rows, r0 + rows_per_block);
+    __shared__ unsigned mxs[4];
     float s = 0.f;
     unsigned mx = 0u;
     if (c < C)
@@ -1300,7 +1301,7 @@
             mx = max(mx, mag_bits(v));
             s += v;
         }
-    if (amax_out) wave_mag_out(mx, amax_out);
+    if (amax_out) block_mag_out(mx, amax_out, mxs);
     if (partial && c < C) partial[(int64_t)blockIdx.x * C + c] = s;
 }
 
@@ -1310,6 +1311,7 @@
                                                               float *__restrict__ amax_out)
 {
     __shared__ float4 red[256];
+    __shared__ unsigned mxs[4];
     unsigned mx = 0u;
     const int C4 = C >> 2;
     const int cbase = blockIdx.y * 256;
@@ -1353,7 +1355,7 @@
             s.x += v.x; s.y += v.y; s.z += v.z; s.w += v.w;
         }
     }
-    if (amax_out) wave_mag_out(mx, amax_out);
+    if (amax_out) block_mag_out(mx, amax_out, mxs);
     if (!partial) return;
     red[threadIdx.x] = s;
     __syncthreads();
diff --git a/htd_amd/csrc/conv_x3.hip b/htd_amd/csrc/conv_x3.hip
--- a/htd_amd/csrc/conv_x3.hip
+++ b/htd_amd/csrc/conv_x3.hip
@@ -117,33 +117,6 @@
     float *amax_out;
 };
 
-__device__ __forceinline__ void block_absmax_out(float mx, float *out, float *red, unsigned seen)
-{
-    unsigned bits = (mx != mx) ? 0x7fc00000u : __float_as_uint(mx);
-    for (int o = 32; o > 0; o >>= 1) bits = max(bits, (unsigned)__shfl_xor((int)bits, o));
-    __syncthreads();
-    if ((threadIdx.x & 63) == 0) reinterpret_cast<unsigned *>(red)[threadIdx.x >> 6] = bits;
-    __syncthreads();
-    if (threadIdx.x == 0) {
-        const unsigned *r = reinterpret_cast<const unsigned *>(red);
-        bits = max(max(r[0], r[1]), max(r[2], r[3]));
-        if (bits > seen) __hip_atomic_fetch_max(reinterpret_cast<unsigned *>(out), bits, __ATOMIC_RELAXED, __HIP_MEMORY_SCOPE_AGENT);
-    }
-}
-__device__ __forceinline__ void wave_absmax_out(float mx, float *out, unsigned seen)
-{
-    unsigned bits = (mx != mx) ? 0x7fc00000u : __float_as_uint(mx);
-    for (int o = 32; o > 0; o >>= 1) bits = max(bits, (unsigned)__shfl_xor((int)bits, o));
-    if ((threadIdx.x & 63) == 0 && bits > seen)
-        __hip_atomic_fetch_max(reinterpret_cast<unsigned *>(out), bits, __ATOMIC_RELAXED, __HIP_MEMORY_SCOPE_AGENT);
-}
-__device__ __forceinline__ float absmax4(float mx, float4 v)
-{
-    const float m = fmaxf(fmaxf(fabsf(v.x), fabsf(v.y)), fmaxf(fabsf(v.z), fabsf(v.w)));
-    const bool nan = (v.x != v.x) | (v.y != v.y) | (v.z != v.z) | (v.w != v.w);
-    return nan ? __uint_as_float(0x7fc00000u) : ((mx != mx) ? mx : fmaxf(mx, m));
-}
-
 __device__ __forceinline__ void emit_planes4(uint4 *yp, int64_t rows, int64_t m, int n, float4 v)
 {
     unsigned h0, m0, l0, h1, m1, l1;
@@ -186,8 +159,7 @@
     float *le = reinterpret_cast<float *>(lds);
     const bool vec_ok = (p.Co & 3) == 0;
     constexpr int V = BN / 4, RPP = 256 / V;
-    float omax = 0.f;
-    const unsigned oseen = (p.amax_out != nullptr && !part) ? *reinterpret_cast<const volatile unsigned *>(p.amax_out) : 0u;
+    unsigned omax = 0u;
     const bool scaled = p.wscale != nullptr;
     float4 cscale = make_float4(1.f, 1.f, 1.f, 1.f);
     if (scaled) {
@@ -268,7 +240,7 @@
                 for (int u = 0; u < UB; ++u)
                     if (ok[u]) {
                         *reinterpret_cast<float4 *>(p.y + o[u]) = v[u];
-                        omax = absmax4(omax, v[u]);
+                        omax = htd::mag_bits4(omax, v[u]);
                     }
                 if (p.yp != nullptr) {
 #pragma unroll
@@ -326,7 +298,7 @@
                     v.z = mv.z > 0.f ? v.z : 0.f; v.w = mv.w > 0.f ? v.w : 0.f;
                 }
                 *reinterpret_cast<float4 *>(p.y + o) = v;
-                omax = absmax4(omax, v);
+                omax = htd::mag_bits4(omax, v);
                 if (p.yp != nullptr) emit_planes4(p.yp, p.yp_rows, m, n, v);
             } else {
                 auto put = [&](int e, float t) {
@@ -336,14 +308,17 @@
                     if (p.relu) t = fmaxf(t, 0.f);
                     if (p.mask_src) t = p.mask_src[o + e] > 0.f ? t : 0.f;
                     p.y[o + e] = t;
-                    omax = absmax4(omax, make_float4(t, 0.f, 0.f, 0.f));
+                    omax = max(omax, htd::mag_bits(t));
                 };
                 put(0, v.x); put(1, v.y); put(2, v.z); put(3, v.w);
             }
         }
         if (i + 1 < TM) __syncthreads();
     }
-    if (p.amax_out != nullptr && !part) block_absmax_out(omax, p.amax_out, le, oseen);
+    if (p.amax_out != nullptr && !part) {
+        __syncthreads();
+        htd::block_mag_out(omax, p.amax_out, reinterpret_cast<unsigned *>(le));
+    }
 }
 
 template <int WGM, int WGN, int TM, int TN, int KW, int NB, bool H2 = false>
@@ -972,8 +947,8 @@
     const int64_t lo = p.splits_a > 1 ? 0 : p.m_rem0 * p.Co, hi = p.splits_b > 1 ? p.M * p.Co : p.m_rem0 * p.Co;
     const int64_t na = p.m_rem0 * p.Co, nb = (p.M - p.m_rem0) * p.Co;
     const float *pb = p.partial + (p.splits_a > 1 ? (int64_t)p.splits_a * na : 0);
-    float omax = 0.f;
-    const unsigned oseen = p.amax_out != nullptr ? *reinterpret_cast<const volatile unsigned *>(p.amax_out) : 0u;
+    __shared__ unsigned ored[4];
+    unsigned omax = 0u;
     for (int64_t o = lo + (int64_t)blockIdx.x * blockDim.x + threadIdx.x; o < hi; o += (int64_t)gridDim.x * blockDim.x) {
         float v = 0.f;
         if (o < na) {
@@ -999,10 +974,9 @@
         const int64_t oo = p.o_step == 0 ? o : x3_out_off(p, o / p.Co, n);
         if (p.mask_src) v = p.mask_src[oo] > 0.f ? v : 0.f;
         p.y[oo] = v;
-        omax = absmax4(omax, make_float4(v, 0.f, 0.f, 0.f));
-    }
-    __shared__ float ored[4];
-    if (p.amax_out != nullptr) block_absmax_out(omax, p.amax_out, ored, oseen);
+        omax = max(omax, htd::mag_bits(v));
+    }
+    if (p.amax_out != nullptr) htd::block_mag_out(omax, p.amax_out, ored);
 }
 
 __global__ __launch_bounds__(256) void conv_x3p_splitk_epilogue_vec_kernel(X3Params p)
@@ -1012,8 +986,8 @@
     const int64_t na = p.m_rem0 * C4, nb = (p.M - p.m_rem0) * C4;
     const float4 *pa = reinterpret_cast<const float4 *>(p.partial);
     const float4 *pb = pa + (p.splits_a > 1 ? (int64_t)p.splits_a * na : 0);
-    float omax = 0.f;
-    const unsigned oseen = p.amax_out != nullptr ? *reinterpret_cast<const volatile unsigned *>(p.amax_out) : 0u;
+    __shared__ unsigned ored[4];
+    unsigned omax = 0u;
     for (int64_t q = lo + (int64_t)blockIdx.x * blockDim.x + threadIdx.x; q < hi; q += (int64_t)gridDim.x * blockDim.x) {
         float4 v = make_float4(0.f, 0.f, 0.f, 0.f);
         const bool in_a = q < na;
@@ -1050,11 +1024,10 @@
             v.z = mv.z > 0.f ? v.z : 0.f; v.w = mv.w > 0.f ? v.w : 0.f;
         }
         *reinterpret_cast<float4 *>(p.y + o) = v;
-        omax = absmax4(omax, v);
+        omax = htd::mag_bits4(omax, v);
         if (p.yp != nullptr) emit_planes4(p.yp, p.yp_rows, (int64_t)m, (int)n, v);
     }
-    __shared__ float ored[4];
-    if (p.amax_out != nullptr) block_absmax_out(omax, p.amax_out, ored, oseen);
+    if (p.amax_out != nullptr) htd::block_mag_out(omax, p.amax_out, ored);
 }
 
 __device__ __forceinline__ void x3_planes_element(const float *__restrict__ w, uint4 *__restrict__ out, int Co, int taps,
@@ -1582,10 +1555,10 @@
     if (pl.partial_floats > 0) {
         const int64_t rows = (p.splits_a > 1 ? p.m_rem0 : 0) + (p.splits_b > 1 ? p.M - p.m_rem0 : 0);
         if ((p.Co & 3) == 0) {
-            const unsigned rb = (unsigned)std::min<int64_t>(htd::ceil_div(rows * (p.Co >> 2), 256), p.amax_out ? 1024 : 4096);
+            const unsigned rb = (unsigned)std::min<int64_t>(htd::ceil_div(rows * (p.Co >> 2), 256), htd::kEmitGrid);
             hipLaunchKernelGGL(conv_x3p_splitk_epilogue_vec_kernel, dim3(rb), dim3(256), 0, s, p);
         } else {
-            const unsigned rb = (unsigned)std::min<int64_t>(htd::ceil_div(rows * p.Co, 256), p.amax_out ? 1024 : 4096);
+            const unsigned rb = (unsigned)std::min<int64_t>(htd::ceil_div(rows * p.Co, 256), htd::kEmitGrid);
             hipLaunchKernelGGL(conv_x3p_splitk_epilogue_kernel, dim3(rb), dim3(256), 0, s, p);
         }
     }
diff --git a/htd_amd/csrc/roi_align.hip b/htd_amd/csrc/roi_align.hip
--- a/htd_amd/csrc/roi_align.hip
+++ b/htd_amd/csrc/roi_align.hip
@@ -220,63 +220,58 @@
                                                                    int sampling_ratio, int aligned, int chunks, int64_t tasks,
                                                                    float *__restrict__ amax_out)
 {
+    __shared__ unsigned mxs[4];
     const int lane = threadIdx.x & 63;
-    const int64_t task = (int64_t)blockIdx.x * (blockDim.x >> 6) + (threadIdx.x >> 6);
-    if (task >= tasks) return;
-    const unsigned seen = amax_out ? *reinterpret_cast<const volatile unsigned *>(amax_out) : 0u;
-    const int chunk = (int)(task % chunks);
-    const int64_t t2 = task / chunks;
-    const int bin = (int)(t2 % (ph * pw));
-    const int64_t ri = t2 / (ph * pw);
-    const int lv = (int)roi_level[ri];
-    const int ch = chunk * 256 + lane * 4;
-    const bool act = ch < C;
-    const size_t bin_off = ((size_t)ri * ph * pw + bin) * C;
-    float4 acc = make_float4(0.f, 0.f, 0.f, 0.f);
-    RoiGeom g{};
-    g.inv_count = 0.f;
-    if (lv >= 0 && lv < L) {
-        const int H = tab.H[lv], W = tab.W[lv];
-        const float *feat = tab.feat[lv];
-        const int bi = bin / pw, bj = bin % pw;
-        g = roi_geometry(rois + 5 * ri, tab.scale[lv], ph, pw, sampling_ratio, aligned);
-        int r0, r1, c0, c1;
-        axis_span(g.start_h, g.bin_h, bi, g.grid_h, H, r0, r1);
-        axis_span(g.start_w, g.bin_w, bj, g.grid_w, W, c0, c1);
-        if (g.batch < 0 || g.batch >= B) { r0 = 0; r1 = -1; }
-        const size_t img_base = (size_t)g.batch * H * W * C;
-        for (int rb = r0; rb <= r1; rb += 64) {
-            const float wy_l = (rb + lane <= r1) ? axis_weight(g.start_h, g.bin_h, bi, g.grid_h, rb + lane, H) : 0.f;
-            for (int cb = c0; cb <= c1; cb += 64) {
-                const float wx_l = (cb + lane <= c1) ? axis_weight(g.start_w, g.bin_w, bj, g.grid_w, cb + lane, W) : 0.f;
-                const int rn = min(64, r1 - rb + 1), cn = min(64, c1 - cb + 1);
-                for (int r = 0; r < rn; ++r) {
-                    const float wy = lane_bcast(wy_l, r);
-                    const float *row = feat + img_base + ((size_t)(rb + r) * W + cb) * C + ch;
+    unsigned mx = 0u;
+    for (int64_t task = (int64_t)blockIdx.x * 4 + (threadIdx.x >> 6); task < tasks; task += (int64_t)gridDim.x * 4) {
+        const int chunk = (int)(task % chunks);
+        const int64_t t2 = task / chunks;
+        const int bin = (int)(t2 % (ph * pw));
+        const int64_t ri = t2 / (ph * pw);
+        const int lv = (int)roi_level[ri];
+        const int ch = chunk * 256 + lane * 4;
+        const bool act = ch < C;
+        const size_t bin_off = ((size_t)ri * ph * pw + bin) * C;
+        float4 acc = make_float4(0.f, 0.f, 0.f, 0.f);
+        RoiGeom g{};
+        g.inv_count = 0.f;
+        if (lv >= 0 && lv < L) {
+            const int H = tab.H[lv], W = tab.W[lv];
+            const float *feat = tab.feat[lv];
+            const int bi = bin / pw, bj = bin % pw;
+            g = roi_geometry(rois + 5 * ri, tab.scale[lv], ph, pw, sampling_ratio, aligned);
+            int r0, r1, c0, c1;
+            axis_span(g.start_h, g.bin_h, bi, g.grid_h, H, r0, r1);
+            axis_span(g.start_w, g.bin_w, bj, g.grid_w, W, c0, c1);
+            if (g.batch < 0 || g.batch >= B) { r0 = 0; r1 = -1; }
+            const size_t img_base = (size_t)g.batch * H * W * C;
+            for (int rb = r0; rb <= r1; rb += 64) {
+                const float wy_l = (rb + lane <= r1) ? axis_weight(g.start_h, g.bin_h, bi, g.grid_h, rb + lane, H) : 0.f;
+                for (int cb = c0; cb <= c1; cb += 64) {
+                    const float wx_l = (cb + lane <= c1) ? axis_weight(g.start_w, g.bin_w, bj, g.grid_w, cb + lane, W) : 0.f;
+                    const int rn = min(64, r1 - rb + 1), cn = min(64, c1 - cb + 1);
+                    for (int r = 0; r < rn; ++r) {
+                        const float wy = lane_bcast(wy_l, r);
+                        const float *row = feat + img_base + ((size_t)(rb + r) * W + cb) * C + ch;
 #pragma unroll 4
-                    for (int c = 0; c < cn; ++c) {
-                        const float w = wy * lane_bcast(wx_l, c);
-                        if (act) {
-                            const float4 v = *reinterpret_cast<const float4 *>(row + (size_t)c * C);
-                            acc.x += w * v.x; acc.y += w * v.y; acc.z += w * v.z; acc.w += w * v.w;
+                        for (int c = 0; c < cn; ++c) {
+                            const float w = wy * lane_bcast(wx_l, c);
+                            if (act) {
+                                const float4 v = *reinterpret_cast<const float4 *>(row + (size_t)c * C);
+                                acc.x += w * v.x; acc.y += w * v.y; acc.z += w * v.z; acc.w += w * v.w;
+                            }
                         }
                     }
                 }
             }
         }
-    }
-    if (act) {
-        acc.x *= g.inv_count; acc.y *= g.inv_count; acc.z *= g.inv_count; acc.w *= g.inv_count;
-        *reinterpret_cast<float4 *>(out + bin_off + ch) = acc;
-    }
-    if (amax_out) {
-        const bool nan = act && ((acc.x != acc.x) | (acc.y != acc.y) | (acc.z != acc.z) | (acc.w != acc.w));
-        const float m = act ? fmaxf(fmaxf(fabsf(acc.x), fabsf(acc.y)), fmaxf(fabsf(acc.z), fabsf(acc.w))) : 0.f;
-        unsigned bits = nan ? 0x7fc00000u : __float_as_uint(m);
-        for (int o = 32; o > 0; o >>= 1) bits = max(bits, (unsigned)__shfl_xor((int)bits, o));
-        if (lane == 0 && bits > seen)
-            __hip_atomic_fetch_max(reinterpret_cast<unsigned *>(amax_out), bits, __ATOMIC_RELAXED, __HIP_MEMORY_SCOPE_AGENT);
-    }
+        if (act) {
+            acc.x *= g.inv_count; acc.y *= g.inv_count; acc.z *= g.inv_count; acc.w *= g.inv_count;
+            *reinterpret_cast<float4 *>(out + bin_off + ch) = acc;
+            mx = htd::mag_bits4(mx, acc);
+        }
+    }
+    if (amax_out) htd::block_mag_out(mx, amax_out, mxs);
 }
 
 struct AllLevelsOut {
@@ -816,8 +811,7 @@
     }
     const int chunks = (C + 255) / 256;
     const int64_t tasks = n * ph * pw * chunks;
-    const int64_t blocks = htd::ceil_div(tasks, 4);
-    HTD_REQUIRE(blocks < (1ll << 31), "roi_align_levels: too many tasks");
+    const int64_t blocks = std::min<int64_t>(htd::ceil_div(tasks, 4), htd::kEmitGrid);
     hipLaunchKernelGGL(roi_align_levels_fwd_kernel, dim3((unsigned)blocks), dim3(256), 0, (hipStream_t)stream, tab, rois, roi_level, out,
                        n, B, C, L, ph, pw, sampling_ratio, aligned, chunks, tasks, amax_out);
     return htd::check_launch("roi_align_levels");
diff --git a/htd_amd/csrc/roi_ops.hip b/htd_amd/csrc/roi_ops.hip
--- a/htd_amd/csrc/roi_ops.hip
+++ b/htd_amd/csrc/roi_ops.hip
@@ -14,6 +14,7 @@
                                                               float *__restrict__ out, int64_t total4, int P,
                                                               int C4, int B, float *__restrict__ amax_out)
 {
+    __shared__ unsigned mxs[4];
     unsigned mx = 0u;
     for (int64_t idx = (int64_t)blockIdx.x * blockDim.x + threadIdx.x; idx < total4;
          idx += (int64_t)gridDim.x * blockDim.x) {
@@ -31,13 +32,14 @@
         st4(out + idx * 4, v);
         mx = htd::mag_bits4(mx, v);
     }
-    if (amax_out) htd::wave_mag_out(mx, amax_out);
+    if (amax_out) htd::block_mag_out(mx, amax_out, mxs);
 }
 
 __global__ __launch_bounds__(256) void plain_and_fused_kernel(const float *__restrict__ x, const float *__restrict__ rois,
                                                               const float *__restrict__ g, float *__restrict__ both,
                                                               int64_t total4, int P, int C4, int B, float *__restrict__ amax_out)
 {
+    __shared__ unsigned mxs[4];
     unsigned mx = 0u;
     for (int64_t idx = (int64_t)blockIdx.x * blockDim.x + threadIdx.x; idx < total4; idx += (int64_t)gridDim.x * blockDim.x) {
         const int c4 = (int)(idx % C4);
@@ -52,7 +54,7 @@
         st4(both + (total4 + idx) * 4, v);
         mx = htd::mag_bits4(mx, v);
     }
-    if (amax_out) htd::wave_mag_out(mx, amax_out);
+    if (amax_out) htd::block_mag_out(mx, amax_out, mxs);
 }
 
 constexpr int ROIS_PER_BLOCK = 16;
@@ -779,7 +781,7 @@
     if (n == 0) return HTD_OK;
     HTD_REQUIRE(roi_feats && rois && global_feat && out, "fuse_global: null pointer");
     const int64_t total4 = n * P * (C / 4);
-    hipLaunchKernelGGL(fuse_global_fwd_kernel, dim3(grid_for(total4)), dim3(256), 0, (hipStream_t)stream, roi_feats,
+    hipLaunchKernelGGL(fuse_global_fwd_kernel, dim3(grid_for(total4, 256, htd::kEmitGrid)), dim3(256), 0, (hipStream_t)stream, roi_feats,
                        rois, global_feat, extra, alpha, out, total4, P, C / 4, B, amax_out);
     return htd::check_launch("fuse_global_fwd");
 }
@@ -805,7 +807,7 @@
     if (n == 0) return HTD_OK;
     HTD_REQUIRE(roi_feats && rois && global_feat && both, "plain_and_fused: null pointer");
     const int64_t total4 = n * P * (C / 4);
-    hipLaunchKernelGGL(plain_and_fused_kernel, dim3(grid_for(total4)), dim3(256), 0, (hipStream_t)stream, roi_feats, rois,
+    hipLaunchKernelGGL(plain_and_fused_kernel, dim3(grid_for(total4, 256, htd::kEmitGrid)), dim3(256), 0, (hipStream_t)stream, roi_feats, rois,
                        global_feat, both, total4, P, C / 4, B, amax_out);
     return htd::check_launch("plain_and_fused_fwd");
 }
@@ -1105,6 +1107,7 @@
                                                            int Wo, int k, int s, int p, float *__restrict__ amax_out)
 {
     const int64_t total = (int64_t)B * Ho * Wo * C4;
+    __shared__ unsigned mxs[4];
     unsigned mx = 0u;
     for (int64_t t = (int64_t)blockIdx.x * 256 + threadIdx.x; t < total; t += (int64_t)gridDim.x * 256) {
         const int c4 = (int)(t % C4);
@@ -1132,7 +1135,7 @@
         if (idx) reinterpret_cast<int4 *>(idx)[t] = am;
         mx = htd::mag_bits4(mx, m);
     }
-    if (amax_out) htd::wave_mag_out(mx, amax_out);
+    if (amax_out) htd::block_mag_out(mx, amax_out, mxs);
 }
 
 __global__ __launch_bounds__(256) void max_pool_bwd_kernel(const float *__restrict__ g, const int *__restrict__ idx,
@@ -1259,7 +1262,7 @@
     const int Ho = (H + 2 * pad - k) / stride + 1, Wo = (W + 2 * pad - k) / stride + 1;
     HTD_REQUIRE(Ho > 0 && Wo > 0, "max_pool2d: empty output");
     const int64_t total = (int64_t)B * Ho * Wo * (C / 4);
-    const unsigned blocks = (unsigned)std::min<int64_t>(htd::ceil_div(total, 256), 65536);
+    const unsigned blocks = (unsigned)std::min<int64_t>(htd::ceil_div(total, 256), htd::kEmitGrid);
     hipLaunchKernelGGL(max_pool_fwd_kernel, dim3(blocks), dim3(256), 0, (hipStream_t)stream, x, y, idx, B, H, W, C / 4,
                        Ho, Wo, k, stride, pad, amax_out);
     return htd::check_launch("max_pool2d_fwd");
```
